# liruiluo/VLA-Adapter

Hardware: AMD Instinct MI355X
Metric: fine-tune samples/sec (224px img + 32-tok prompt), adapter-only, fwd+bwd+AdamW (higher is better)
Workload: dtype bf16

## Files before the change

### vla_adapter_amd/csrc/common.h

```cpp
#pragma once
#include <hip/hip_runtime.h>
#include <stdint.h>
#include <stdio.h>

typedef unsigned short bf16_t;
typedef __attribute__((ext_vector_type(8))) short bf16x8;
typedef __attribute__((ext_vector_type(4))) short bf16x4;
typedef __attribute__((ext_vector_type(4))) float f32x4;
typedef __attribute__((ext_vector_type(16))) float f32x16;
typedef __attribute__((ext_vector_type(4))) unsigned u32x4;
typedef __attribute__((ext_vector_type(8))) int v8i_f8;

#define VLA_OK 0
#define VLA_ERR_ARG (-1)
#define VLA_ERR_LAUNCH (-2)
#define VLA_ERR_UNSUPPORTED (-3)

extern "C" void vla_set_error(const char* msg);

#define VLA_REQUIRE(cond, msg)            \
  do {                                    \
    if (!(cond)) {                        \
      vla_set_error(msg);                 \
      return VLA_ERR_ARG;                 \
// ... 39 lines not shown
}
__device__ __forceinline__ void unpack8(const uint4& u, float (&f)[8]) {
  const unsigned w[4] = {u.x, u.y, u.z, u.w};
#pragma unroll
  for (int k = 0; k < 4; ++k) {
    f[2 * k] = bf_lo(w[k]);
    f[2 * k + 1] = bf_hi(w[k]);
  }
}
template <class V>
__device__ __forceinline__ uint2 pack4(const V& f) { return uint2{pack2(f[0], f[1]), pack2(f[2], f[3])}; }
__device__ __forceinline__ uint4 pack8(const float (&f)[8]) {
  return uint4{pack2(f[0], f[1]), pack2(f[2], f[3]), pack2(f[4], f[5]), pack2(f[6], f[7])};
}

__device__ __forceinline__ unsigned long long splitmix64_key(unsigned long long seed, unsigned long long idx) {
  unsigned long long z = seed + idx * 0x9E3779B97F4A7C15ull;
  z = (z ^ (z >> 30)) * 0xBF58476D1CE4E5B9ull;
  z = (z ^ (z >> 27)) * 0x94D049BB133111EBull;
  return z ^ (z >> 31);
}

__device__ __forceinline__ long long action_token_id(float v, const double* __restrict__ bins, int nbins, float lo, float hi,
                                                     long long tokenizer_len) {
  const double x = (double)fminf(fmaxf(v, lo), hi);
  int a = 0, b = nbins;
  while (a < b) {
    const int mid = (a + b) >> 1;
    if (bins[mid] <= x) a = mid + 1;
    else b = mid;
  }
  return tokenizer_len - a;
}

__device__ __forceinline__ float wave_sum(float v) {
#pragma unroll
  for (int o = 32; o > 0; o >>= 1) v += __shfl_xor(v, o, 64);
  return v;
}
__device__ __forceinline__ float wave_max(float v) {
#pragma unroll
  for (int o = 32; o > 0; o >>= 1) v = fmaxf(v, __shfl_xor(v, o, 64));
  return v;
}

__device__ __forceinline__ float fast_erf(float x) {
  const float ax = fabsf(x);
  const float t = __builtin_amdgcn_rcpf(1.0f + 0.3275911f * ax);
  const float poly = t * (0.254829592f + t * (-0.284496736f + t * (1.421413741f + t * (-1.453152027f + t * 1.061405429f))));
  const float r = 1.0f - poly * __expf(-ax * ax);
  return copysignf(r, x);
}
__device__ __forceinline__ float gelu_erf(float x) {
  const float ax = fabsf(x);
  const float t = __builtin_amdgcn_rcpf(__builtin_fmaf(ax, 0.3275911f * 0.70710678118654752440f, 1.0f));
  const float poly = t * (0.127414796f + t * (-0.142248368f + t * (0.7107068705f + t * (-0.7265760135f + t * 0.5307027145f))));
  const float e = __builtin_amdgcn_exp2f(x * x * -0.72134752044448170368f);
  return __builtin_fmaf(-ax * poly, e, fmaxf(x, 0.f));
}
__device__ __forceinline__ float gelu_erf_grad(float x) {
  const float c = 0.3989422804014327f;
  return 0.5f * (1.0f + fast_erf(x * 0.70710678118654752440f)) + x * c * __expf(-0.5f * x * x);
}
__device__ __forceinline__ float gelu_tanh(float x) {
  const float u2 = x * __builtin_fmaf(x * x, 0.044715f * 1.5957691216057308f, 1.5957691216057308f);
  return x * __builtin_amdgcn_rcpf(1.0f + __builtin_amdgcn_exp2f(u2 * -1.4426950408889634f));
}

__device__ __forceinline__ void lds_zero16(void* p, int bytes, int idx, int n) {
  for (int i = idx * 16; i < bytes; i += n * 16) *reinterpret_cast<uint4*>(reinterpret_cast<char*>(p) + i) = uint4{0, 0, 0, 0};
}

__device__ __forceinline__ void glds16(const void* gptr, void* lds_wave_base) {
  __builtin_amdgcn_global_load_lds((const __attribute__((address_space(1))) void*)gptr,
                                   (__attribute__((address_space(3))) void*)lds_wave_base, 16, 0, 0);
}

__device__ __forceinline__ void glds16s(const char* base, unsigned voff, unsigned dst) {
  unsigned keep;
  asm volatile("s_mov_b32 %0, m0\n\ts_mov_b32 m0, %3\n\ts_nop 0\n\tglobal_load_lds_dwordx4 %1, %2\n\ts_mov_b32 m0, %0"
               : "=&s"(keep) : "v"(voff), "s"(base), "s"(dst) : "memory");
}

__device__ __forceinline__ v8i_f8 cat8(bf16x8 lo, bf16x8 hi) {
  typedef float f32x8 __attribute__((ext_vector_type(8)));
  const f32x4 l = __builtin_bit_cast(f32x4, lo), h = __builtin_bit_cast(f32x4, hi);
  return __builtin_bit_cast(v8i_f8, f32x8{l[0], l[1], l[2], l[3], h[0], h[1], h[2], h[3]});
}

#define VLA_BARRIER()                      \
  do {                                     \
    __builtin_amdgcn_sched_barrier(0);     \
    __builtin_amdgcn_s_barrier();          \
    asm volatile("" ::: "memory");         \
    __builtin_amdgcn_sched_barrier(0);     \
  } while (0)

__device__ __forceinline__ int xcd_order(int bid, int nwg) {
  const int xcd = bid & 7, q8 = nwg >> 3, r8 = nwg & 7;
  return (xcd < r8 ? xcd * (q8 + 1) : r8 * (q8 + 1) + (xcd - r8) * q8) + (bid >> 3);
}

constexpr int CR_THREADS = 1024;

template <int LPR>
struct CR {
  static constexpr int COLS = 8 * LPR, GROUPS = CR_THREADS / LPR;
  static __device__ __forceinline__ int col() { return blockIdx.x * COLS + (threadIdx.x % LPR) * 8; }
  static __device__ __forceinline__ int row0() { return threadIdx.x / LPR; }
  static int blocks(int cols) { return (cols + COLS - 1) / COLS; }

  static __device__ __forceinline__ void add(float (&a)[8], float* __restrict__ out, int cols, float (*sm)[64]) {
    const int lane = threadIdx.x & 63, w = threadIdx.x >> 6;
#pragma unroll
    for (int k = 0; k < 8; ++k)
#pragma unroll
      for (int o = LPR; o < 64; o <<= 1) a[k] += __shfl_xor(a[k], o, 64);
    if (lane < LPR)
#pragma unroll
      for (int k = 0; k < 8; ++k) sm[w][lane * 8 + k] = a[k];
    __syncthreads();
    const int c = blockIdx.x * COLS + threadIdx.x;
    if (threadIdx.x < COLS && c < cols) {
      float s = 0.f;
#pragma unroll
      for (int i = 0; i < CR_THREADS / 64; ++i) s += sm[i][threadIdx.x];
      atomicAdd(out + c, s);
    }
    __syncthreads();
  }
};

#define CR_LAUNCH(KERNEL, rows, cols, batch, stream, ...) \
  hipLaunchKernelGGL(KERNEL<8>, dim3(CR<8>::blocks(cols), 1, (batch)), dim3(CR_THREADS), 0, (hipStream_t)(stream), __VA_ARGS__)
```

### vla_adapter_amd/csrc/elementwise.hip

```cpp
#include "gemm_epilogue.h"
#include "argmax_order.h"
#include <type_traits>

namespace {

inline unsigned nblk(long long n, int per) { return (unsigned)((n + per - 1) / per); }

__global__ void im2col_kernel(const void* __restrict__ px, bf16_t* __restrict__ out, int B, int Ctot, int c0, int H,
                              int W, int P, int ldo, int f32in) {
  const int gw = W / P, gh = H / P, KK = 3 * P * P;
  const long long total = (long long)B * gh * gw * ldo;
  for (long long i = (long long)blockIdx.x * blockDim.x + threadIdx.x; i < total; i += (long long)gridDim.x * blockDim.x) {
    const int col = i % ldo;
    const long long prow = i / ldo;
    float v = 0.f;
    if (col < KK) {
      const int c = col / (P * P), rem = col - c * P * P, py = rem / P, pxx = rem - py * P;
      const int pw = prow % gw, ph = (prow / gw) % gh, b = prow / ((long long)gw * gh);
      const long long src = (((long long)b * Ctot + c0 + c) * H + ph * P + py) * W + pw * P + pxx;
      v = f32in ? ((const float*)px)[src] : bf2f(((const bf16_t*)px)[src]);
    }
    out[i] = f2bf(v);
  }
}

__global__ void action_mask_kernel(const long long* __restrict__ labels, int* __restrict__ qidx, int* __restrict__ pos,
                                   int* __restrict__ count, int B, int L, int shift) {
  const int b = blockIdx.x, lane = threadIdx.x;
  const long long* row = labels + (long long)b * L + shift;
  const int n = L - shift;
  int base = 0;
  for (int j0 = 0; j0 < n; j0 += 64) {
    const int j = j0 + lane;
    const bool sel = j < n && row[j] != -100 && row[j] > 151386;
    const unsigned long long bal = __ballot(sel);
    const int k = base + __popcll(bal & ((1ull << lane) - 1ull));
    if (j < n) qidx[(long long)b * n + j] = sel ? k : -1;
    if (sel && k < 64) pos[b * 64 + k] = j;
    base += __popcll(bal);
  }
  if (lane == 0) count[b] = base;
  for (int k = base + lane; k < 64; k += 64) pos[b * 64 + k] = -1;
}

__global__ void embed_splice_kernel(const long long* __restrict__ ids, const unsigned char* __restrict__ am,
                                    const int* __restrict__ qidx, const bf16_t* __restrict__ table,
                                    const bf16_t* __restrict__ aq, bf16_t* __restrict__ out,
                                    unsigned char* __restrict__ mm, int B, int L, int Np, int D, int vocab) {
  const int S = L + Np;
  const int lane = threadIdx.x & 63;
  const long long r = (long long)blockIdx.x * 4 + (threadIdx.x >> 6);
  if (r >= (long long)B * S) return;
  const int b = r / S, s = r - (long long)b * S;
  if (s >= 1 && s <= Np) {
    if (lane == 0 && mm) mm[r] = 1;
    return;
  }
  const int j = s == 0 ? 0 : s - Np;
  const int qi = qidx[(long long)b * L + j];
  long long id = ids[(long long)b * L + j];
  if (id < 0 || id >= vocab) id = 0;
  const bf16_t* src = qi >= 0 ? aq + (long long)min(qi, 63) * D : table + id * D;
  bf16_t* dst = out + r * D;
  for (int e = lane * 8; e < D; e += 512) *reinterpret_cast<uint4*>(dst + e) = *reinterpret_cast<const uint4*>(src + e);
  if (lane == 0 && mm) mm[r] = am ? (am[(long long)b * L + j] != 0) : 1;
}

__global__ void action_query_grad_kernel(const bf16_t* __restrict__ dx, const int* __restrict__ pos, float* __restrict__ dq,
                                         int B, int S, int Np, int D, int row0) {
  const int k = blockIdx.x;
  for (int d = threadIdx.x; d < D; d += blockDim.x) {
    float a = 0.f;
    for (int b = 0; b < B; ++b) {
      const int j = pos[b * 64 + k];
      if (j < 0) continue;
      const int s = (j == 0 ? 0 : Np + j) - row0;
      if (s < 0) continue;
      a += bf2f(dx[((long long)b * S + s) * D + d]);
    }
    dq[k * D + d] = a;
  }
}

__global__ void gather_rows_kernel(const bf16_t* __restrict__ in, const int* __restrict__ idx, bf16_t* __restrict__ out,
// ... 58 lines not shown
#pragma unroll
    for (int k = 0; k < 8; ++k) {
      const float sg = 1.f / (1.f + __expf(-g[k]));
      du[k] = d[k] * (g[k] * sg);
      dg[k] = d[k] * u[k] * silu_grad(g[k], sg);
    }
    *reinterpret_cast<uint4*>(dgu + go) = pack8(dg);
    *reinterpret_cast<uint4*>(dgu + go + 16) = pack8(du);
  }
}

__global__ __launch_bounds__(256) void transpose_kernel(const bf16_t* __restrict__ in, bf16_t* __restrict__ out, int rows,
                                                        int cols, int ldi, int ldo, long long s_in, long long s_out) {
  __shared__ bf16_t t[64][66];
  const bf16_t* ib = in + (long long)blockIdx.z * s_in;
  bf16_t* ob = out + (long long)blockIdx.z * s_out;
  const int r0 = blockIdx.y * 64, c0 = blockIdx.x * 64;
  const int tx = threadIdx.x & 63, ty = threadIdx.x >> 6;
  for (int r = ty; r < 64; r += 4)
    t[r][tx] = (r0 + r < rows && c0 + tx < cols) ? ib[(long long)(r0 + r) * ldi + c0 + tx] : (bf16_t)0;
  __syncthreads();
  for (int c = ty; c < 64; c += 4)
    if (c0 + c < cols && r0 + tx < rows) ob[(long long)(c0 + c) * ldo + r0 + tx] = t[tx][c];
}

__global__ __launch_bounds__(256) void transpose_vec_kernel(const bf16_t* __restrict__ in, bf16_t* __restrict__ out, int rows,
                                                            int cols, int ldi, int ldo, long long s_in, long long s_out) {
  __shared__ unsigned t32[64 * 33];
  const bf16_t* ib = in + (long long)blockIdx.z * s_in;
  bf16_t* ob = out + (long long)blockIdx.z * s_out;
  const int r0 = blockIdx.y * 64, c0 = blockIdx.x * 64;
  for (int i = threadIdx.x; i < 512; i += 256) {
    const int r = i >> 3, ch = i & 7;
    uint4 v = {0u, 0u, 0u, 0u};
    if (r0 + r < rows && c0 + ch * 8 < cols) v = *reinterpret_cast<const uint4*>(ib + (long long)(r0 + r) * ldi + c0 + ch * 8);
    unsigned* d = t32 + r * 33 + ch * 4;
    d[0] = v.x; d[1] = v.y; d[2] = v.z; d[3] = v.w;
  }
  __syncthreads();
  const bf16_t* t = reinterpret_cast<const bf16_t*>(t32);
  for (int i = threadIdx.x; i < 512; i += 256) {
    const int g = i & 7, c = i >> 3;
    if (c0 + c < cols && r0 + g * 8 < rows) {
      unsigned o[4];
#pragma unroll
      for (int k = 0; k < 4; ++k)
        o[k] = (unsigned)t[(g * 8 + 2 * k) * 66 + c] | ((unsigned)t[(g * 8 + 2 * k + 1) * 66 + c] << 16);
      *reinterpret_cast<uint4*>(ob + (long long)(c0 + c) * ldo + r0 + g * 8) = uint4{o[0], o[1], o[2], o[3]};
    }
  }
}

__global__ void colsum_kernel(const bf16_t* __restrict__ x, float* __restrict__ out, int rows, int cols, int ldx, long long s_x,
                              long long s_out) {
  const int c = blockIdx.x * 256 + threadIdx.x;
  if (c >= cols) return;
  x += (long long)blockIdx.z * s_x;
  out += (long long)blockIdx.z * s_out;
  float a = 0.f;
  for (int r = 0; r < rows; ++r) a += bf2f(x[(long long)r * ldx + c]);
  atomicAdd(out + c, a);
}

template <int LPR>
__global__ __launch_bounds__(CR_THREADS) void colsum_vec_kernel(const bf16_t* __restrict__ x, float* __restrict__ out, int rows, int cols,
                                                                int ldx, long long s_x, long long s_out) {
  __shared__ float sm[CR_THREADS / 64][64];
  const int c = CR<LPR>::col();
  x += (long long)blockIdx.z * s_x;
  out += (long long)blockIdx.z * s_out;
  float a[8] = {0, 0, 0, 0, 0, 0, 0, 0};
  if (c < cols)
    for (int r = CR<LPR>::row0(); r < rows; r += CR<LPR>::GROUPS) {
      float f[8];
      unpack8(*reinterpret_cast<const uint4*>(x + (long long)r * ldx + c), f);
#pragma unroll
      for (int k = 0; k < 8; ++k) a[k] += f[k];
    }
  CR<LPR>::add(a, out, cols, sm);
}

__global__ void cast_f32_bf16_kernel(const float* __restrict__ x, bf16_t* __restrict__ y, long long n) {
  for (long long i = (long long)blockIdx.x * blockDim.x + threadIdx.x; i < n; i += (long long)gridDim.x * blockDim.x) y[i] = f2bf(x[i]);
}
__global__ void cast_bf16_f32_kernel(const bf16_t* __restrict__ x, float* __restrict__ y, long long n) {
  for (long long i = (long long)blockIdx.x * blockDim.x + threadIdx.x; i < n; i += (long long)gridDim.x * blockDim.x) y[i] = bf2f(x[i]);
}

__global__ void rope_half_kernel(bf16_t* __restrict__ x, const float* __restrict__ ct, const float* __restrict__ st, long long rows,
                                 int S, int nheads, int dh, int ldx, float sign) {
  const int half = dh / 2;
  const long long total = rows * nheads * half;
  for (long long i = (long long)blockIdx.x * blockDim.x + threadIdx.x; i < total; i += (long long)gridDim.x * blockDim.x) {
    const int d = i % half;
    const long long t = i / half;
    const int hh = t % nheads;
    const long long r = t / nheads;
    const int pos = r % S;
    bf16_t* p = x + r * ldx + hh * dh + d;
    const float a = bf2f(p[0]), b = bf2f(p[half]);
    const float c = ct[pos * half + d], s = sign * st[pos * half + d];
    p[0] = f2bf(rope_rot_a(a, b, c, s));
    p[half] = f2bf(rope_rot_b(a, b, c, s));
  }
}

__global__ void rope_inter_kernel(bf16_t* __restrict__ x, const float* __restrict__ ct, const float* __restrict__ st,
                                  long long rows, int T, int nheads, int dh, int ldx, int mode) {
  const int half = dh / 2;
  const long long total = rows * nheads * half;
  for (long long i = (long long)blockIdx.x * blockDim.x + threadIdx.x; i < total; i += (long long)gridDim.x * blockDim.x) {
    const int d = i % half;
    const long long t = i / half;
    const int hh = t % nheads;
    const long long r = t / nheads;
    const int pos = r % T;
    bf16_t* p = x + r * ldx + hh * dh + 2 * d;
    const float a = bf2f(p[0]), b = bf2f(p[1]);
    const float ca = ct[pos * dh + 2 * d], cb = ct[pos * dh + 2 * d + 1];
    const float sa = st[pos * dh + 2 * d], sb = st[pos * dh + 2 * d + 1];
    if (mode == 0) {
      p[0] = f2bf(rope_rot_a(a, b, ca, sa));
      p[1] = f2bf(rope_rot_b(a, b, cb, sb));
    } else {
      p[0] = f2bf(a * ca + b * sb);
      p[1] = f2bf(b * cb - a * sa);
    }
  }
}

__global__ void rope_inter_vec_kernel(bf16_t* __restrict__ x, const float* __restrict__ ct, const float* __restrict__ st,
                                      int rows, int T, int nheads, int dh, int ldx, int mode) {
  const int cpr = nheads * dh / 8;
  const long long total = (long long)rows * cpr;
  for (long long i = (long long)blockIdx.x * blockDim.x + threadIdx.x; i < total; i += (long long)gridDim.x * blockDim.x) {
    const int r = (int)(i / cpr), col = (int)(i - (long long)r * cpr) * 8;
    const int d0 = col % dh, pos = r % T;
    uint4* px = reinterpret_cast<uint4*>(x + (long long)r * ldx + col);
    float f[8], o[8];
    unpack8(*px, f);
    const float4 c0 = *reinterpret_cast<const float4*>(ct + (long long)pos * dh + d0), c1 = *reinterpret_cast<const float4*>(ct + (long long)pos * dh + d0 + 4);
    const float4 s0 = *reinterpret_cast<const float4*>(st + (long long)pos * dh + d0), s1 = *reinterpret_cast<const float4*>(st + (long long)pos * dh + d0 + 4);
    const float cc[8] = {c0.x, c0.y, c0.z, c0.w, c1.x, c1.y, c1.z, c1.w}, ss[8] = {s0.x, s0.y, s0.z, s0.w, s1.x, s1.y, s1.z, s1.w};
#pragma unroll
    for (int k = 0; k < 8; k += 2) {
      const float a = f[k], b = f[k + 1];
      if (mode == 0) {
        o[k] = rope_rot_a(a, b, cc[k], ss[k]);
        o[k + 1] = rope_rot_b(a, b, cc[k + 1], ss[k + 1]);
      } else {
        o[k] = a * cc[k] + b * ss[k + 1];
        o[k + 1] = b * cc[k + 1] - a * ss[k];
      }
    }
    *px = pack8(o);
  }
}

__global__ __launch_bounds__(256) void l1_loss_kernel(const bf16_t* __restrict__ pred, const bf16_t* __restrict__ tgt,
                                                      float* __restrict__ loss3, bf16_t* __restrict__ dpred, int B, int C,
                                                      int Da, float gscale) {
  __shared__ float red[3][4];
  const int n = B * C * Da;
  float a = 0.f, cur = 0.f, nxt = 0.f;
  for (int i = threadIdx.x; i < n; i += 256) {
    const float d = bf2f(pred[i]) - bf2f(tgt[i]);
// ... 209 lines not shown
  hipLaunchKernelGGL(action_query_grad_kernel, dim3(64), dim3(256), 0, (hipStream_t)stream, (const bf16_t*)dx, pos, dq, B, S, Np, D, row0);
  VLA_CHECK_LAUNCH("action_query_grad");
  return VLA_OK;
}

extern "C" int vla_gather_rows(void* stream, const void* in, const int* idx, void* out, int n, int D, int ldi, int ldo) {
  VLA_REQUIRE(in && idx && out && n > 0 && D % 8 == 0 && ldi % 8 == 0 && ldo % 8 == 0, "gather_rows: bad args");
  VLA_REQUIRE(((((uintptr_t)in) | ((uintptr_t)out)) & 15) == 0, "gather_rows: 16-B aligned in / out");
  hipLaunchKernelGGL(gather_rows_kernel, dim3(nblk(n, 4)), dim3(256), 0, (hipStream_t)stream, (const bf16_t*)in, idx, (bf16_t*)out, n, D, ldi, ldo);
  VLA_CHECK_LAUNCH("gather_rows");
  return VLA_OK;
}

extern "C" int vla_scatter_add_rows(void* stream, const void* in, const int* idx, void* out, int n, int D, int ldi, int ldo) {
  VLA_REQUIRE(in && idx && out && n > 0 && D % 8 == 0 && ldi % 8 == 0 && ldo % 8 == 0, "scatter_add_rows: bad args");
  VLA_REQUIRE(((((uintptr_t)in) | ((uintptr_t)out)) & 15) == 0, "scatter_add_rows: 16-B aligned in / out");
  hipLaunchKernelGGL(scatter_add_rows_kernel, dim3(nblk(n, 4)), dim3(256), 0, (hipStream_t)stream, (const bf16_t*)in, idx, (bf16_t*)out, n, D, ldi, ldo);
  VLA_CHECK_LAUNCH("scatter_add_rows");
  return VLA_OK;
}

#define EW_ENTRY(NAME, OP, NEEDB)                                                                                  \
  extern "C" int NAME(void* stream, const void* a, const void* b, void* y, long long n) {                           \
    VLA_REQUIRE(a && y && (!(NEEDB) || b) && n > 0 && n % 8 == 0, #NAME ": null / n%8");                              \
    VLA_REQUIRE(((((uintptr_t)a) | ((uintptr_t)b) | ((uintptr_t)y)) & 15) == 0, #NAME ": 16-B aligned tensors");     \
    hipLaunchKernelGGL(ew_kernel<OP>, GRID1D(n / 8, 256), dim3(256), 0, (hipStream_t)stream, (const bf16_t*)a,     \
                       (const bf16_t*)b, (bf16_t*)y, n / 8);                                                       \
    VLA_CHECK_LAUNCH(#NAME);                                                                                       \
    return VLA_OK;                                                                                                 \
  }
EW_ENTRY(vla_add_bf16, EW_ADD, 1)
EW_ENTRY(vla_gelu_bwd, EW_GELU_B, 1)
EW_ENTRY(vla_relu_bwd, EW_RELU_B, 1)
extern "C" int vla_gelu_fwd(void* stream, const void* x, void* y, long long n) {
  VLA_REQUIRE(x && y && n > 0 && n % 8 == 0, "gelu_fwd: null / n%8");
  VLA_REQUIRE(((((uintptr_t)x) | ((uintptr_t)y)) & 15) == 0, "gelu_fwd: 16-B aligned tensors");
  hipLaunchKernelGGL(ew_kernel<EW_GELU_F>, GRID1D(n / 8, 256), dim3(256), 0, (hipStream_t)stream, (const bf16_t*)x,
                     (const bf16_t*)nullptr, (bf16_t*)y, n / 8);
  VLA_CHECK_LAUNCH("gelu_fwd");
  return VLA_OK;
}

extern "C" int vla_swiglu_bwd(void* stream, const void* dh, const void* gu, void* dgu, int M, int I) {
  VLA_REQUIRE(dh && gu && dgu && M > 0 && I > 0 && I % 16 == 0, "swiglu_bwd: I%16");
  VLA_REQUIRE(((((uintptr_t)dh) | ((uintptr_t)gu) | ((uintptr_t)dgu)) & 15) == 0, "swiglu_bwd: 16-B aligned tensors");
  const long long nch = (long long)M * (I / 8);
  hipLaunchKernelGGL(swiglu_bwd_kernel, GRID1D(nch, 256), dim3(256), 0, (hipStream_t)stream, (const bf16_t*)dh, (const bf16_t*)gu, (bf16_t*)dgu, nch, I);
  VLA_CHECK_LAUNCH("swiglu_bwd");
  return VLA_OK;
}

extern "C" int vla_transpose_bf16(void* stream, const void* in, void* out, int rows, int cols, int ldi, int ldo, int batch,
                                  long long s_in, long long s_out) {
  VLA_REQUIRE(in && out && rows > 0 && cols > 0 && ldi >= cols && ldo >= rows && batch > 0, "transpose: bad args");
  dim3 grid((cols + 63) / 64, (rows + 63) / 64, batch);
  const bool vec = rows % 8 == 0 && cols % 8 == 0 && ldi % 8 == 0 && ldo % 8 == 0 && s_in % 8 == 0 && s_out % 8 == 0 &&
                   ((((uintptr_t)in) | ((uintptr_t)out)) & 15) == 0;
  if (vec)
    hipLaunchKernelGGL(transpose_vec_kernel, grid, dim3(256), 0, (hipStream_t)stream, (const bf16_t*)in, (bf16_t*)out, rows, cols, ldi, ldo, s_in, s_out);
  else
    hipLaunchKernelGGL(transpose_kernel, grid, dim3(256), 0, (hipStream_t)stream, (const bf16_t*)in, (bf16_t*)out, rows, cols, ldi, ldo, s_in, s_out);
  VLA_CHECK_LAUNCH("transpose");
  return VLA_OK;
}

extern "C" int vla_colsum_bf16(void* stream, const void* x, float* out, int rows, int cols, int ldx, int batch, long long s_x,
                               long long s_out) {
  VLA_REQUIRE(x && out && rows > 0 && cols > 0 && ldx >= cols && batch > 0, "colsum: bad args");
  if (cols % 8 == 0 && ldx % 8 == 0 && s_x % 8 == 0 && ((uintptr_t)x & 15) == 0) {
    CR_LAUNCH(colsum_vec_kernel, rows, cols, batch, stream, (const bf16_t*)x, out, rows, cols, ldx, s_x, s_out);
    VLA_CHECK_LAUNCH("colsum");
    return VLA_OK;
  }
  hipLaunchKernelGGL(colsum_kernel, dim3((cols + 255) / 256, 1, batch), dim3(256), 0, (hipStream_t)stream, (const bf16_t*)x, out, rows,
                     cols, ldx, s_x, s_out);
  VLA_CHECK_LAUNCH("colsum");
  return VLA_OK;
}

extern "C" int vla_cast_f32_bf16(void* stream, const float* x, void* y, long long n) {
  VLA_REQUIRE(x && y && n > 0, "cast: bad args");
  hipLaunchKernelGGL(cast_f32_bf16_kernel, GRID1D(n, 256), dim3(256), 0, (hipStream_t)stream, x, (bf16_t*)y, n);
  VLA_CHECK_LAUNCH("cast_f32_bf16");
  return VLA_OK;
}
extern "C" int vla_cast_bf16_f32(void* stream, const void* x, float* y, long long n) {
  VLA_REQUIRE(x && y && n > 0, "cast: bad args");
  hipLaunchKernelGGL(cast_bf16_f32_kernel, GRID1D(n, 256), dim3(256), 0, (hipStream_t)stream, (const bf16_t*)x, y, n);
  VLA_CHECK_LAUNCH("cast_bf16_f32");
  return VLA_OK;
}

extern "C" int vla_rope_half(void* stream, void* x, const float* cos_t, const float* sin_t, int rows, int S, int nheads, int dh,
                             int ldx, int sign) {
  VLA_REQUIRE(x && cos_t && sin_t && rows > 0 && S > 0 && nheads > 0 && dh % 2 == 0 && ldx >= nheads * dh, "rope_half: bad args");
  const long long total = (long long)rows * nheads * (dh / 2);
  hipLaunchKernelGGL(rope_half_kernel, GRID1D(total, 256), dim3(256), 0, (hipStream_t)stream, (bf16_t*)x, cos_t, sin_t, (long long)rows, S, nheads, dh, ldx, sign >= 0 ? 1.f : -1.f);
  VLA_CHECK_LAUNCH("rope_half");
  return VLA_OK;
}

extern "C" int vla_rope_interleaved(void* stream, void* x, const float* cos_t, const float* sin_t, int rows, int T, int nheads,
                                    int dh, int ldx, int mode) {
  VLA_REQUIRE(x && cos_t && sin_t && rows > 0 && T > 0 && nheads > 0 && dh % 2 == 0 && ldx >= nheads * dh, "rope_interleaved: bad args");
  const long long total = (long long)rows * nheads * (dh / 2);
  if (dh % 8 == 0 && ldx % 8 == 0 && (((uintptr_t)x | (uintptr_t)cos_t | (uintptr_t)sin_t) & 15) == 0) {
    const long long tv = (long long)rows * (nheads * dh / 8);
    hipLaunchKernelGGL(rope_inter_vec_kernel, GRID1D(tv, 256), dim3(256), 0, (hipStream_t)stream, (bf16_t*)x, cos_t, sin_t, (int)rows, T, nheads, dh, ldx, mode);
  } else
  hipLaunchKernelGGL(rope_inter_kernel, GRID1D(total, 256), dim3(256), 0, (hipStream_t)stream, (bf16_t*)x, cos_t, sin_t, (long long)rows, T, nheads, dh, ldx, mode);
  VLA_CHECK_LAUNCH("rope_interleaved");
  return VLA_OK;
}

extern "C" int vla_l1_loss(void* stream, const void* pred, const void* target, float* loss3, void* dpred, int B, int C, int Da,
                           float gscale) {
  VLA_REQUIRE(pred && target && loss3 && B > 0 && C > 0 && Da > 0, "l1_loss: bad args");
  hipLaunchKernelGGL(l1_loss_kernel, dim3(1), dim3(256), 0, (hipStream_t)stream, (const bf16_t*)pred, (const bf16_t*)target, loss3, (bf16_t*)dpred, B, C, Da, gscale);
  VLA_CHECK_LAUNCH("l1_loss");
  return VLA_OK;
}

static int adamw_launch(void* stream, void* p, const void* g, void* m, void* v, long long n, double lr, double beta1, double beta2,
                        double eps, double wd, int step, int g_f32, float gscale, const float* coef) {
  VLA_REQUIRE(p && g && m && v && n > 0 && step >= 1, "adamw: bad args");
  const double bc1 = 1.0 - pow(beta1, step), bc2 = 1.0 - pow(beta2, step);
  const float decay = (float)(1.0 - lr * wd);
  const float omb1 = (float)(1.0 - beta1), omb2 = (float)(1.0 - beta2);
  const float neg_step = (float)(-(lr / bc1));
  const float gs = gscale == 0.f ? 1.f : gscale;
  const bool aligned = ((((uintptr_t)p) | ((uintptr_t)g) | ((uintptr_t)m) | ((uintptr_t)v)) & 15) == 0;
  const long long n8 = aligned ? n / 8 : 0, done = n8 * 8;
  if (n8 > 0)
    hipLaunchKernelGGL(coef ? adamw_vec8_kernel<true> : adamw_vec8_kernel<false>, GRID1D(n8, 256), dim3(256), 0, (hipStream_t)stream,
                       (uint4*)p, g, (uint4*)m, (uint4*)v, n8, decay, omb1, (float)beta2, omb2, (float)sqrt(bc2), (float)eps, neg_step,
                       g_f32, gs, coef);
  if (done < n)
    hipLaunchKernelGGL(coef ? adamw_kernel<true> : adamw_kernel<false>, GRID1D(n - done, 256), dim3(256), 0, (hipStream_t)stream,
                       (bf16_t*)p + done, g_f32 ? (const void*)((const float*)g + done) : (const void*)((const bf16_t*)g + done),
                       (bf16_t*)m + done, (bf16_t*)v + done, n - done, decay, omb1, (float)beta2, omb2, (float)sqrt(bc2), (float)eps,
                       neg_step, g_f32, gs, coef);
  VLA_CHECK_LAUNCH("adamw");
  return VLA_OK;
}

extern "C" int vla_adamw_bf16(void* stream, void* p, const void* g, void* m, void* v, long long n, double lr, double beta1,
                              double beta2, double eps, double wd, int step, int g_f32, float gscale) {
  return adamw_launch(stream, p, g, m, v, n, lr, beta1, beta2, eps, wd, step, g_f32, gscale, nullptr);
}

extern "C" int vla_adamw_clipped_bf16(void* stream, void* p, const void* g, void* m, void* v, long long n, double lr, double beta1,
                                      double beta2, double eps, double wd, int step, int g_f32, float gscale, const float* coef) {
  VLA_REQUIRE(coef, "adamw_clipped: null coefficient");
  return adamw_launch(stream, p, g, m, v, n, lr, beta1, beta2, eps, wd, step, g_f32, gscale, coef);
}

extern "C" long long vla_grad_sumsq_slots(long long n) { return n > 0 ? (n + GRAD_SSQ_CHUNK - 1) / GRAD_SSQ_CHUNK : 0; }

extern "C" int vla_grad_sumsq(void* stream, const void* g, long long n, int g_f32, float gscale, float* slots) {
  VLA_REQUIRE(g && slots && n > 0, "grad_sumsq: bad args");
  VLA_REQUIRE(((uintptr_t)g & (g_f32 ? 3 : 1)) == 0 && ((uintptr_t)slots & 3) == 0, "grad_sumsq: misaligned pointer");
  const long long nb = vla_grad_sumsq_slots(n);
  VLA_REQUIRE(nb <= 0x7fffffffLL, "grad_sumsq: slice too long");
  const float gs = gscale == 0.f ? 1.f : gscale;
  hipLaunchKernelGGL(g_f32 ? grad_sumsq_kernel<true> : grad_sumsq_kernel<false>, dim3((unsigned)nb), dim3(256), 0, (hipStream_t)stream, g, n, gs, slots);
  VLA_CHECK_LAUNCH("grad_sumsq");
// ... 643 lines not shown
```

### vla_adapter_amd/csrc/gemm.hip

```cpp
#include <algorithm>
#include "gemm_epilogue.h"
#include "gemm_params.h"

namespace {

constexpr int BK = 64;
constexpr int EPI_PAD = 16;

__device__ __forceinline__ float apply_act(float v, int act) {
  switch (act) {
    case VLA_ACT_GELU: return rbf(gelu_erf(v));
    case VLA_ACT_RELU: return fmaxf(v, 0.f);
    case VLA_ACT_GELU_TANH: return rbf(gelu_tanh(v));
    default: return v;
  }
}

template <int BM, int BN, int STAGES, int WN = 2>
struct Cfg {
  static constexpr int NW = (BM / 64) * WN;
  static constexpr int NTHREADS = NW * 64;
  static constexpr int WTN = BN / WN;
  static constexpr int NT = WTN / 16;
  static constexpr int A_BYTES = BM * BK * 2, B_BYTES = BN * BK * 2;
  static constexpr int STAGE_BYTES = A_BYTES + B_BYTES;
  static constexpr int PIECES = STAGE_BYTES / 1024;
  static constexpr int PPW = PIECES / NW;
  static constexpr int EPI_STRIDE = WTN * 2 + EPI_PAD;
  static constexpr int LDS_BYTES = STAGES * STAGE_BYTES;
  static constexpr int NHALF = NW * 64 * EPI_STRIDE <= LDS_BYTES ? 1 : 2;
  static constexpr int EPI_ROWS = 64 / NHALF;
  static constexpr int EPI_BYTES = NW * EPI_ROWS * EPI_STRIDE;
  static_assert(EPI_BYTES <= LDS_BYTES, "epilogue staging must fit the operand ring");
  static_assert(PIECES % NW == 0, "pieces must divide evenly over the waves");
};

template <int BM, int BN, int STAGES, int ROPE, int WN = 2, bool F8 = false, bool EXT = false>
__global__ __launch_bounds__((BM / 64) * 64 * WN) __attribute__((amdgpu_waves_per_eu((F8 && EXT) ? 4 : 1)))
void gemm_nt_kernel(GemmP p) {
  using C = Cfg<BM, BN, STAGES, WN>;
  constexpr int EB = F8 ? 1 : 2;
  extern __shared__ __attribute__((aligned(16))) char smem[];
  const int tid = threadIdx.x, lane = tid & 63;
  const int wid = __builtin_amdgcn_readfirstlane(tid >> 6);
  const int wr = wid / WN, wc = wid - wr * WN;

  const int swz = xcd_order(blockIdx.x, p.ntiles);
  constexpr int GM = 6;
  const int tiles_m = p.ntiles / p.tiles_n, per_group = GM * p.tiles_n;
  const int grp = swz / per_group, rem = swz - grp * per_group;
  const int gm = min(GM, tiles_m - grp * GM);
  const int bm = grp * GM + rem % gm, bn = rem / gm;
  const int m0 = bm * BM, n0 = bn * BN;
  const int z = blockIdx.z;
  const char* Ab = reinterpret_cast<const char*>(p.A) + (long long)z * p.sA * EB;
  const char* Bb = reinterpret_cast<const char*>(p.B) + (long long)z * p.sB * EB;

  const int kc = ((lane & 7) ^ ((lane >> 3) & 7)) * 16;
  const char* pp[C::PPW];
#pragma unroll
  for (int i = 0; i < C::PPW; ++i) {
    const int pc = wid * C::PPW + i;
    if (pc < BM / 8) {
      const int ra = min(m0 + pc * 8 + (lane >> 3), p.M - 1);
      pp[i] = Ab + grouped_row(ra, p.gA, p.sgA, p.lda) * EB + kc;
    } else {
      const int rb = min(n0 + (pc - BM / 8) * 8 + (lane >> 3), p.N - 1);
      pp[i] = Bb + (long long)rb * p.ldb * EB + kc;
    }
  }
  const char* pp2[EXT ? C::PPW : 1];
  if constexpr (EXT) {
#pragma unroll
    for (int i = 0; i < C::PPW; ++i) {
      const int pc = wid * C::PPW + i;
      if (pc < BM / 8) pp2[i] = reinterpret_cast<const char*>(p.A2) + (long long)min(m0 + pc * 8 + (lane >> 3), p.M - 1) * p.lda2 * 2 + kc;
      else pp2[i] = reinterpret_cast<const char*>(p.B2) + (long long)min(n0 + (pc - BM / 8) * 8 + (lane >> 3), p.N - 1) * p.ldb2 * 2 + kc;
    }
  }
  const int nt1 = (p.Ktot > 0 ? min(p.K, p.Ktot - z * p.K) : p.K) / (F8 ? 2 * BK : BK);
  auto stage = [&](int buf, int t) {
    char* base = smem + buf * C::STAGE_BYTES + wid * C::PPW * 1024;
    if (EXT && t >= nt1) {
#pragma unroll
      for (int i = 0; i < C::PPW; ++i) glds16(pp2[i] + (t - nt1) * 128, base + i * 1024);
    } else {
#pragma unroll
      for (int i = 0; i < C::PPW; ++i) glds16(pp[i] + t * 128, base + i * 1024);
    }
  };

  f32x4 acc[C::NT][4];
#pragma unroll
  for (int a = 0; a < C::NT; ++a)
#pragma unroll
    for (int b = 0; b < 4; ++b) acc[a][b] = f32x4{0.f, 0.f, 0.f, 0.f};

  const int frow = lane & 15;
  int foff[2], foff2[2];
#pragma unroll
  for (int s = 0; s < 2; ++s) {
    foff[s] = frow * 128 + (((F8 ? 2 * (lane >> 4) + s : 4 * s + (lane >> 4)) ^ (lane & 7)) << 4);
    foff2[s] = frow * 128 + (((4 * s + (lane >> 4)) ^ (lane & 7)) << 4);
  }

  const int wm0 = m0 + wr * 64, wn0 = n0 + wc * C::WTN;
  const int lq = lane >> 4, lr = lane & 15;
  constexpr bool PERM = ROPE == 1 && C::NT == 2;
  const bool wide = PERM && p.rope_dh == 128;
  auto cbase = [&](int ni) { return PERM ? (wide ? ni * 64 + wc * 16 : (wc >> 1) * 64 + ni * 32 + (wc & 1) * 16) : wc * C::WTN + ni * 16; };
  const bf16_t* bias = p.bias ? p.bias + (long long)z * p.sBias : nullptr;
  float bv[C::NT][4];
  {
    const bool bvec = bias && (((size_t)bias & 7) == 0);
#pragma unroll
    for (int ni = 0; ni < C::NT; ++ni) {
      const int n = n0 + cbase(ni) + lq * 4;
      if (bvec && n + 3 < p.N) {
        const uint2 b2 = *reinterpret_cast<const uint2*>(bias + n);
        bv[ni][0] = bf_lo(b2.x); bv[ni][1] = bf_hi(b2.x);
        bv[ni][2] = bf_lo(b2.y); bv[ni][3] = bf_hi(b2.y);
      } else {
#pragma unroll
        for (int j = 0; j < 4; ++j) bv[ni][j] = (bias && n + j < p.N) ? bf2f(bias[n + j]) : 0.f;
      }
    }
  }

  const int nt = nt1 + (EXT ? p.K2 / BK : 0);
#pragma unroll
  for (int s = 0; s < STAGES - 1; ++s)
    if (s < nt) stage(s, s);
  int buf = 0;
  static_assert(C::NT <= 4, "wave tiles are 64 x 32 or 64 x 64");
  static_assert(STAGES >= 2 && STAGES <= 6 && 4 * C::PPW < 64, "the counted waits below cover rings of 2 to 6 stages (vmcnt is a 6-bit counter)");
#define VLA_KTILE(F8T, FO)                                                                                                           \
  do {                                                                                                                               \
           \
    if (STAGES >= 6 && t + 4 < nt) asm volatile("s_waitcnt vmcnt(%0)" ::"n"(4 * C::PPW) : "memory");                                  \
    else if (STAGES >= 5 && t + 3 < nt) asm volatile("s_waitcnt vmcnt(%0)" ::"n"(3 * C::PPW) : "memory");                             \
    else if (STAGES >= 4 && t + 2 < nt) asm volatile("s_waitcnt vmcnt(%0)" ::"n"(2 * C::PPW) : "memory");                             \
    else if (STAGES >= 3 && t + 1 < nt) asm volatile("s_waitcnt vmcnt(%0)" ::"n"(C::PPW) : "memory");                                 \
    else asm volatile("s_waitcnt vmcnt(0)" ::: "memory");                                                                            \
    __builtin_amdgcn_s_barrier();                     \
    asm volatile("" ::: "memory");                                                                                                   \
    if (t + STAGES - 1 < nt) {                                                                                                       \
      int nb = buf + STAGES - 1;                                                                                                     \
      if (nb >= STAGES) nb -= STAGES;                                                                                                \
      stage(nb, t + STAGES - 1);                                                                                                     \
    }                                                                                                                                \
    const char* sa = smem + buf * C::STAGE_BYTES + wr * 64 * 128;                                                                    \
    const char* sb = smem + buf * C::STAGE_BYTES + C::A_BYTES;              \
    bf16x8 fm[2][4], fn[2][C::NT];                                                                                                   \
    _Pragma("unroll") for (int s = 0; s < 2; ++s) {                                                                                  \
      _Pragma("unroll") for (int i = 0; i < 4; ++i) fm[s][i] = *reinterpret_cast<const bf16x8*>(sa + i * 16 * 128 + FO[s]);          \
      _Pragma("unroll") for (int i = 0; i < C::NT; ++i) fn[s][i] = *reinterpret_cast<const bf16x8*>(sb + cbase(i) * 128 + FO[s]);    \
    }                                                                                                                                \
    if constexpr (F8T) {                                                                                                             \
      _Pragma("unroll") for (int ni = 0; ni < C::NT; ++ni)                                                                           \
        _Pragma("unroll") for (int mi = 0; mi < 4; ++mi)                                                                             \
          acc[ni][mi] = __builtin_amdgcn_mfma_scale_f32_16x16x128_f8f6f4(cat8(fn[0][ni], fn[1][ni]), cat8(fm[0][mi], fm[1][mi]),     \
                                                                         acc[ni][mi], 0, 0, 0, 0x7f7f7f7f, 0, 0x7f7f7f7f);            \
    } else {                                                                                                                         \
      _Pragma("unroll") for (int s = 0; s < 2; ++s)                                                                                  \
        _Pragma("unroll") for (int ni = 0; ni < C::NT; ++ni)                                                                         \
          _Pragma("unroll") for (int mi = 0; mi < 4; ++mi)                                                                           \
            acc[ni][mi] = __builtin_amdgcn_mfma_f32_16x16x32_bf16(fn[s][ni], fm[s][mi], acc[ni][mi], 0, 0, 0);                       \
    }                                                                                                                                \
    if (++buf == STAGES) buf = 0;                                                                                                    \
  } while (0)
  if constexpr (F8 && EXT) {
    for (int t = 0; t < nt1; ++t) VLA_KTILE(true, foff);
    {
      float fsa[4];
#pragma unroll
      for (int mi = 0; mi < 4; ++mi) fsa[mi] = p.scaleA[min(wm0 + mi * 16 + lr, p.M - 1)];
#pragma unroll
      for (int ni = 0; ni < C::NT; ++ni)
#pragma unroll
        for (int j = 0; j < 4; ++j) {
          const float sbv = p.scaleB[min(n0 + cbase(ni) + lq * 4 + j, p.N - 1)];
#pragma unroll
          for (int mi = 0; mi < 4; ++mi) acc[ni][mi][j] *= fsa[mi] * sbv;
        }
    }
    for (int t = nt1; t < nt; ++t) VLA_KTILE(false, foff2);
  } else {
    for (int t = 0; t < nt; ++t) VLA_KTILE(F8, foff);
  }
#undef VLA_KTILE
  asm volatile("s_waitcnt lgkmcnt(0)" ::: "memory");
  __builtin_amdgcn_s_barrier();
  asm volatile("" ::: "memory");

  if constexpr (F8 && !EXT) {
    float sa[4];
#pragma unroll
    for (int mi = 0; mi < 4; ++mi) sa[mi] = p.scaleA[min(wm0 + mi * 16 + lr, p.M - 1)];
#pragma unroll
    for (int ni = 0; ni < C::NT; ++ni) {
      const int n = n0 + cbase(ni) + lq * 4;
#pragma unroll
      for (int j = 0; j < 4; ++j) {
        const float sbv = p.scaleB[min(n + j, p.N - 1)];
#pragma unroll
        for (int mi = 0; mi < 4; ++mi) acc[ni][mi][j] *= sa[mi] * sbv;
      }
    }
  }
  if (ROPE == 0 && p.ws != nullptr) {
    float* plane = p.ws + (long long)z * p.M * p.N;
#pragma unroll
    for (int ni = 0; ni < C::NT; ++ni)
#pragma unroll
      for (int mi = 0; mi < 4; ++mi) {
        const int m = wm0 + mi * 16 + lr, n = wn0 + ni * 16 + lq * 4;
        if (m < p.M && n + 3 < p.N)
          *reinterpret_cast<f32x4*>(plane + (long long)m * p.N + n) = acc[ni][mi];
      }
    return;
  }
  char* reg = smem + wid * (C::EPI_ROWS * C::EPI_STRIDE);

  if (ROPE == 3) {
    const bf16_t* GU = p.R + (long long)z * p.sR;
    bf16_t* Cb = p.C + (long long)z * p.sC;
    constexpr int ROWB = 2 * C::WTN * 2 + 16;
    constexpr int CH2 = 2 * C::WTN / 8, RPP2 = 64 / CH2;
    constexpr int NIT = 32 / RPP2;
    char* reg2 = smem + wid * (32 * ROWB);
    if (wn0 >= p.N || wm0 >= p.M) return;
    u32x4 gin[2][NIT];
#pragma unroll
    for (int half = 0; half < 2; ++half)
#pragma unroll
      for (int it = 0; it < NIT; ++it) {
        const int row = it * RPP2 + lane / CH2, ch = lane % CH2;
        const int m = min(wm0 + half * 32 + row, p.M - 1);
        gin[half][it] = *reinterpret_cast<const u32x4*>(GU + grouped_row(m, p.gR, p.sgR, p.ldr) + 2 * wn0 + ch * 8);
// ... 136 lines not shown
            const int row = it * RPP + row0;
            const uint4 v = *reinterpret_cast<const uint4*>(reg + row * C::EPI_STRIDE + ch * 16);
            *reinterpret_cast<uint4*>(Cb + (long long)(wmh + row) * p.ldc + n) = add_packed8(v, rv[it]);
          }
        } else {
#pragma unroll
          for (int it = 0; it < NIT; ++it) {
            const int row = it * RPP + row0;
            *reinterpret_cast<uint4*>(Cb + (long long)(wmh + row) * p.ldc + n) = *reinterpret_cast<const uint4*>(reg + row * C::EPI_STRIDE + ch * 16);
          }
        }
        continue;
      }
    }
#pragma unroll
    for (int it = 0; it < C::EPI_ROWS / RPP; ++it) {
      const int row = it * RPP + lane / CH, ch = lane % CH;
      const int m = wm0 + half * C::EPI_ROWS + row, n = n0 + cbase(ch >> 1) + (ch & 1) * 8;
      uint4 v = *reinterpret_cast<const uint4*>(reg + row * C::EPI_STRIDE + ch * 16);
      if (m >= p.M || n >= p.N) continue;
      if (!row_live(m, p.c_live_mod, p.c_live_from)) continue;
      const long long roff = residual_row(m, p.res_mod, p.gR, p.sgR, p.ldr);
      const long long crow = grouped_row(m, p.gC, p.sgC, p.ldc);
      if (vec_ok && n + 8 <= p.N) {
        if (Rb) v = add_packed8(v, *reinterpret_cast<const uint4*>(Rb + roff + n));
        *reinterpret_cast<uint4*>(Cb + crow + n) = v;
      } else {
        const unsigned wv[4] = {v.x, v.y, v.z, v.w};
#pragma unroll
        for (int k = 0; k < 8; ++k) {
          if (n + k < p.N) {
            float f = (k & 1) ? bf_hi(wv[k >> 1]) : bf_lo(wv[k >> 1]);
            if (Rb) f += bf2f(Rb[roff + n + k]);
            Cb[crow + n + k] = f2bf(f);
          }
        }
      }
    }
  }
}

__global__ void splitk_finalize_kernel(const float* __restrict__ ws, const bf16_t* __restrict__ bias, const bf16_t* __restrict__ R,
                                       bf16_t* __restrict__ C, int M, int N, int ldc, int ldr, int act, float alpha, int split, int vec) {
  const long long total = (long long)M * N / 4, plane = (long long)M * N;
  for (long long i = (long long)blockIdx.x * blockDim.x + threadIdx.x; i < total; i += (long long)gridDim.x * blockDim.x) {
    const int m = (int)(i * 4 / N), n = (int)(i * 4 - (long long)m * N);
    f32x4 pv[8];
#pragma unroll
    for (int z = 0; z < 8; ++z) pv[z] = z < split ? *reinterpret_cast<const f32x4*>(ws + z * plane + i * 4) : f32x4{0.f, 0.f, 0.f, 0.f};
    uint2 braw = {0, 0}, rraw = {0, 0};
    if (vec) {
      if (bias) braw = *reinterpret_cast<const uint2*>(bias + n);
      if (R) rraw = *reinterpret_cast<const uint2*>(R + (long long)m * ldr + n);
    } else {
      if (bias) braw = uint2{(unsigned)bias[n] | ((unsigned)bias[n + 1] << 16), (unsigned)bias[n + 2] | ((unsigned)bias[n + 3] << 16)};
      if (R) {
        const bf16_t* rp = R + (long long)m * ldr + n;
        rraw = uint2{(unsigned)rp[0] | ((unsigned)rp[1] << 16), (unsigned)rp[2] | ((unsigned)rp[3] << 16)};
      }
    }
    f32x4 a = pv[0];
#pragma unroll
    for (int z = 1; z < 8; ++z) a += pv[z];
    for (int z = 8; z < split; ++z) a += *reinterpret_cast<const f32x4*>(ws + z * plane + i * 4);
    const float bb[4] = {bf_lo(braw.x), bf_hi(braw.x), bf_lo(braw.y), bf_hi(braw.y)};
    const float rr[4] = {bf_lo(rraw.x), bf_hi(rraw.x), bf_lo(rraw.y), bf_hi(rraw.y)};
    float o[4];
#pragma unroll
    for (int j = 0; j < 4; ++j) {
      float v = epi_linear(a[j], alpha, bias ? bb[j] : 0.f);
      if (act != VLA_ACT_NONE) v = apply_act(rbf(v), act);
      if (R) v = rbf(v) + rr[j];
      o[j] = v;
    }
    if (vec) {
      *reinterpret_cast<uint2*>(C + (long long)m * ldc + n) = pack4(o);
    } else {
#pragma unroll
      for (int j = 0; j < 4; ++j) C[(long long)m * ldc + n + j] = f2bf(o[j]);
    }
  }
}

template <int BM, int BN, int STAGES, int ROPE, int WN = 2, bool F8 = false, bool EXT = false>
int launch(const GemmP& p0, int nb, hipStream_t st) {
  using C = Cfg<BM, BN, STAGES, WN>;
  if (int rc = vla_lds_limit<gemm_nt_kernel<BM, BN, STAGES, ROPE, WN, F8, EXT>>(C::LDS_BYTES, "gemm_nt_kernel")) return rc;
  GemmP p = p0;
  p.tiles_n = (p.N + BN - 1) / BN;
  p.ntiles = ((p.M + BM - 1) / BM) * p.tiles_n;
  hipLaunchKernelGGL((gemm_nt_kernel<BM, BN, STAGES, ROPE, WN, F8, EXT>), dim3(p.ntiles, 1, nb), dim3(C::NTHREADS), C::LDS_BYTES, st, p);
  return VLA_OK;
}

template <int ROPE, bool F8 = false, bool EXT = false>
int launch_nt(int kernel, const GemmP& p, int nb, hipStream_t st) {
  if constexpr (!F8 && !EXT && ROPE != 3) {
    if (kernel == VLA_KERNEL_NT_64x128_S6) return launch<64, 128, 6, ROPE, 4>(p, nb, st);
    if (kernel == VLA_KERNEL_NT_128x128_S4) return launch<128, 128, 4, ROPE, 4>(p, nb, st);
    if constexpr (ROPE != 1)
      if (kernel == VLA_KERNEL_NT_128x64) return launch<128, 64, 2, ROPE>(p, nb, st);
  }
  return launch<128, 128, 2, ROPE, 4, F8, EXT>(p, nb, st);
}

struct NtOverrides {
  int tile;
  bool no_skinny, no_small_rows, no_splitk, grid_set;
  long long grid;
};
NtOverrides nt_overrides() {
  const char* tile = getenv("VLA_GEMM_TILE");
  const char* nsk = getenv("VLA_NO_SPLITK");
  const char* grid = getenv("VLA_GEMM256_GRID");
  return {tile ? atoi(tile) : 0, getenv("VLA_NO_SKINNY") != nullptr, getenv("VLA_NO_SMALL_ROWS") != nullptr, nsk && *nsk,
          grid != nullptr, grid ? atoll(grid) : 0};
}

thread_local int g_latency_hint = 0;

bool use_256(int M, int N, int K, int batch, int act, int ncu) {
  const long long tiles = (long long)((M + 255) / 256) * ((N + 255) / 256) * batch;
  if (act == VLA_ACT_SWIGLU_BWD) return false;
  if ((act == VLA_ACT_GELU || act == VLA_ACT_GELU_TANH) && tiles > ncu && (tiles % ncu) != 0 && (tiles % ncu) * 4 < ncu) return false;
  const long long t128 = (long long)((M + 127) / 128) * ((N + 127) / 128) * batch;
  const double est256 = (double)((tiles + ncu - 1) / ncu) * 4.0, est128 = (double)((t128 + 2 * ncu - 1) / (2 * ncu)) * (2.0 / 0.87);
  return M >= 1024 && N >= 768 && K >= 256 && est256 < est128;
}

int skinny_tile(const vla_gemm_desc* d, bool latency, int ncu, bool no_small_rows) {
  const bool tall = (d->N == 64 || d->N == 128 || d->N == 192) && d->M >= 1024;
  const bool shortm = latency && d->M <= 512 && d->N % 16 == 0 && d->K >= 512 && !no_small_rows;
  if (!(tall || shortm) || d->K % 128 != 0 || d->K >= 2048 || d->ldc % 8 != 0 || ((uintptr_t)d->C & 15) != 0) return -1;
  if (!(d->act == VLA_ACT_NONE || d->act == VLA_ACT_GELU || d->act == VLA_ACT_RELU || d->act == VLA_ACT_GELU_TANH)) return -1;
  if (d->bias && ((uintptr_t)d->bias & 15) != 0) return -1;
  if (d->R && (d->ldr % 8 != 0 || ((uintptr_t)d->R & 15) != 0)) return -1;
  if ((d->rope_mode == 1 && (d->rope_dh != 64 || d->rope_cols % 64 != 0 || tall)) ||
      (d->rope_mode == 2 && (d->rope_dh % 8 != 0 || d->rope_cols % 8 != 0 || (((uintptr_t)d->rope_cos | (uintptr_t)d->rope_sin) & 15) != 0)))
    return -1;
  int best = -1;
  long long best_cost = 0;
  for (int t = 0; t < SKINNY_TILES; ++t) {
    const int tm = 16 * SKINNY_TILE[t][0], tn = 16 * SKINNY_TILE[t][1];
    if (tall && d->N % tn != 0) continue;
    if (d->rope_mode == 1 && tn != 64) continue;
    const long long wgs = (long long)((d->M + tm - 1) / tm) * ((d->N + tn - 1) / tn), cost = (long long)(tm + tn) * ((wgs + ncu - 1) / ncu);
    if (best < 0 || cost < best_cost || (cost == best_cost && t > best)) best = t, best_cost = cost;
  }
  if (!tall && best_cost > 96) return -1;
  return best;
}

bool ext_on_256(const vla_gemm_desc* d, int force, int ncu) {
  if (d->fp8 || d->batch != 1 || d->split_k > 1 || d->act == VLA_ACT_SWIGLU_BWD || d->rope_mode == 2 || d->a_group != 0 ||
      (d->rope_mode == 1 && d->rope_dh != 64) || !vla_gemm256_extent_ok(d))
    return false;
  const unsigned long long ra = (unsigned long long)((d->M + 255) / 256) * 256, rb = (unsigned long long)((d->N + 255) / 256) * 256;
  if ((ra * d->lda2 + d->K2) * 2 >= (1ull << 32) || (rb * d->ldb2 + d->K2) * 2 >= (1ull << 32)) return false;
  if (force != 0) return force == 6;
  const long long t256 = (long long)((d->M + 255) / 256) * ((d->N + 255) / 256);
  if (d->rope_mode == 1 && t256 < 192) return false;
  return use_256(d->M, d->N, d->K + d->K2, 1, d->act, ncu);
}

struct NtPlan { int kernel, split; };

NtPlan plan_nt(const vla_gemm_desc* d, bool latency, int ncu, const NtOverrides& ov) {
  const int force = ov.tile, kt = d->K / BK;
  const int asked = d->split_k > 1 ? d->split_k : 1, per = (kt + asked - 1) / asked, split = (kt + per - 1) / per;
  if (force == 0 && !ov.no_skinny && d->batch == 1 && split == 1 && d->a_group == 0 && d->c_group == 0 && d->r_group == 0 &&
      d->res_mod == 0 && d->c_live_mod == 0 && !d->fp8 && d->K2 == 0 && d->C) {
    const int t = skinny_tile(d, latency, ncu, ov.no_small_rows);
    if (t >= 0) return {VLA_KERNEL_NT_SKINNY + t, 1};
  }
  const bool fits256 = vla_gemm256_extent_ok(d) != 0;
  if (d->K2 > 0) return {!d->fp8 && ext_on_256(d, force, ncu) ? VLA_KERNEL_NT_256 : VLA_KERNEL_NT_128x128, 1};
  if (d->fp8) {
    const bool big = force == 6 || (force == 0 && d->M >= 4096 && d->N >= 4096 && d->K >= 4096);
    return {big && d->c_group == 0 && d->r_group == 0 && fits256 && !(d->rope_mode == 1 && d->rope_dh != 64) ? VLA_KERNEL_NT_256
                                                                                                              : VLA_KERNEL_NT_128x128, 1};
  }
  const int nb = asked > 1 ? asked : d->batch;
  bool square = false;
  if (asked == 1) {
    const long long t256 = (long long)((d->M + 255) / 256) * ((d->N + 255) / 256) * nb;
    if (force == 6 || (force == 0 && (d->rope_mode == 0 || t256 >= 192) && use_256(d->M, d->N, d->K, nb, d->act, ncu))) {
      if (fits256 && !(d->rope_mode == 2 && (d->R || d->act != VLA_ACT_NONE)) && !(d->rope_mode == 1 && d->rope_dh != 64))
        return {VLA_KERNEL_NT_256, 1};
      square = true;
    }
  }
  if (d->act == VLA_ACT_SWIGLU_BWD) return {VLA_KERNEL_NT_128x128, split};
  const long long tiles = (long long)((d->M + 127) / 128) * ((d->N + 127) / 128) * nb;
  const bool narrow = !square && d->rope_mode != 1 && force != 2 && (force == 3 || (tiles <= 128 && d->K / asked >= 4096 && d->N % 64 == 0));
  if (narrow) return {VLA_KERNEL_NT_128x64, split};
  if (latency && per >= 4) {
    const int runs = split > 1 ? split : d->batch;
    const long long wgs = (long long)((d->M + 127) / 128) * ((d->N + 127) / 128) * runs, wgs64 = (long long)((d->M + 63) / 64) * ((d->N + 127) / 128) * runs;
    if (wgs64 <= ncu) return {VLA_KERNEL_NT_64x128_S6, split};
    if (wgs <= ncu) return {VLA_KERNEL_NT_128x128_S4, split};
  }
  return {VLA_KERNEL_NT_128x128, split};
}

int auto_split_k(const vla_gemm_desc* d, bool latency, int ncu, const NtOverrides& ov) {
  const bool plain = !d->fp8 && d->K2 == 0 && d->batch == 1 && !d->bias_post_round && d->C && d->a_group == 0 && d->c_group == 0 &&
                     d->r_group == 0 && d->rope_mode == 0 && d->c_live_mod == 0 && d->res_mod == 0 && d->N % 4 == 0 &&
                     (d->act == VLA_ACT_NONE || d->act == VLA_ACT_GELU || d->act == VLA_ACT_RELU || d->act == VLA_ACT_GELU_TANH);
  if (!plain || d->K < 2048 || ov.no_splitk) return 1;
  const long long tiles = (long long)((d->M + 127) / 128) * ((d->N + 127) / 128), t64 = (long long)((d->M + 63) / 64) * ((d->N + 127) / 128);
  if (latency && t64 * 2 <= ncu) return (int)std::max(2LL, std::min({ncu / t64, (long long)(d->K / BK) / 4, 16LL}));
  if (tiles > ncu) return 1;
  for (int sk = 8; sk >= 2; sk /= 2)
    if (tiles * sk <= 2 * ncu && d->K % (BK * sk) == 0 && d->K / sk >= 512) return sk;
  return 1;
}

int splitk_finalize(const vla_gemm_desc* d, int split, hipStream_t st) {
  const long long total = (long long)d->M * d->N / 4;
  const unsigned nblk = (unsigned)((total + 255) / 256 < 2048 ? (total + 255) / 256 : 2048);
  hipLaunchKernelGGL(splitk_finalize_kernel, dim3(nblk), dim3(256), 0, st, (const float*)d->ws, (const bf16_t*)d->bias,
                     (const bf16_t*)d->R, (bf16_t*)d->C, d->M, d->N, d->ldc, d->ldr, d->act, d->alpha == 0.f ? 1.f : d->alpha, split,
                     (d->ldc % 4 == 0 && ((uintptr_t)d->C & 7) == 0 && (!d->R || (d->ldr % 4 == 0 && ((uintptr_t)d->R & 7) == 0)) &&
                      (!d->bias || ((uintptr_t)d->bias & 7) == 0)) ? 1 : 0);
  VLA_CHECK_LAUNCH("gemm_splitk_finalize");
  return VLA_OK;
}

}

extern "C" int vla_gemm256_extent_ok(const vla_gemm_desc* d) {
  if (!d || d->M <= 0 || d->N <= 0 || d->K <= 0) return 0;
  const unsigned long long EB = d->fp8 ? 1 : 2, lim = 1ull << 32;
  const unsigned long long ra = (unsigned long long)((d->M + 255) / 256) * 256 - 1, rb = (unsigned long long)((d->N + 255) / 256) * 256 - 1;
  const unsigned long long offA = d->a_group > 0 ? (ra / d->a_group) * (unsigned long long)d->a_group_stride + (ra % d->a_group) * (unsigned long long)d->lda
                                                 : ra * (unsigned long long)d->lda;
  const unsigned long long offB = rb * (unsigned long long)d->ldb;
  return (offA + d->K) * EB < lim && (offB + d->K) * EB < lim;
}

extern "C" int vla_gemm_latency_hint(int on) {
  const int prev = g_latency_hint;
  if (on >= 0) g_latency_hint = on ? 1 : 0;
  return prev;
}

extern "C" int vla_gemm_nt_plan(const vla_gemm_desc* d, int latency, int num_cus, int* split) {
  if (!d || d->M <= 0 || d->N <= 0 || d->K < BK || d->batch <= 0) return VLA_ERR_ARG;
  const bool lat = latency < 0 ? g_latency_hint > 0 : latency > 0;
  const int ncu = num_cus > 0 ? num_cus : vla_num_cus();
  const NtOverrides ov = nt_overrides();
  const NtPlan pl = plan_nt(d, lat, ncu, ov);
  if (split) *split = d->split_k > 1 ? pl.split : auto_split_k(d, lat, ncu, ov);
  return pl.kernel;
}

extern "C" int vla_gemm_bf16_nt(void* stream, const vla_gemm_desc* d) {
  VLA_REQUIRE(d && d->A && d->B, "gemm: null operand");
  VLA_REQUIRE(d->M > 0 && d->N > 0 && d->K > 0 && d->batch > 0, "gemm: empty problem");
  VLA_REQUIRE(d->K % BK == 0, "gemm: K must be a multiple of 64 (pad the operands)");
  VLA_REQUIRE(d->lda % 8 == 0 && d->ldb % 8 == 0, "gemm: lda/ldb must be multiples of 8 elements (16-B rows)");
  if (d->fp8)
    VLA_REQUIRE(d->fp8 == 1 && d->a_scale && d->b_scale && d->K % 128 == 0 && d->lda % 16 == 0 && d->ldb % 16 == 0 && d->batch == 1 &&
                    d->split_k <= 1 && d->rope_mode != 2 && d->a_group == 0 && (d->act != VLA_ACT_SWIGLU_BWD || d->K2 > 0),
                "gemm: fp8 needs scales, K % 128 == 0, 16-B rows, batch 1, no split-K / interleaved RoPE / row groups on A (SwiGLU backward: with a K extension only)");
  VLA_REQUIRE(((uintptr_t)d->A & 15) == 0 && ((uintptr_t)d->B & 15) == 0, "gemm: A/B must be 16-B aligned");
  VLA_REQUIRE(d->sA % 8 == 0 && d->sB % 8 == 0, "gemm: batch strides of A/B must keep 16-B alignment");
  if (d->act == VLA_ACT_SWIGLU_BWD) {
    VLA_REQUIRE(d->C && d->R && !d->bias && d->rope_mode == 0 && d->N % 64 == 0 && d->ldc % 8 == 0 && d->ldr % 4 == 0 &&
                    ((uintptr_t)d->R & 7) == 0 && d->c_group == 0 && d->res_mod == 0,
                "gemm: swiglu_bwd needs C = dGU [M, 2N] (ldc%8), R = GU [M, 2N] (interleaved), N%64 == 0");
  } else if (d->act == VLA_ACT_SWIGLU) {
    VLA_REQUIRE(d->C2 && d->N % 32 == 0 && d->ldc2 % 4 == 0 && ((uintptr_t)d->C2 & 7) == 0 && d->sC2 % 4 == 0,
                "gemm: swiglu needs C2, N%32==0, ldc2%4==0");
    VLA_REQUIRE(!d->R, "gemm: swiglu epilogue takes no residual");
  } else {
    VLA_REQUIRE(d->C, "gemm: null C");
  }
  if (d->C) VLA_REQUIRE(((uintptr_t)d->C & 15) == 0 || (d->ldc % 8) != 0, "gemm: C must be 16-B aligned");
  if (d->C && d->ldc % 8 == 0) VLA_REQUIRE(d->sC % 8 == 0, "gemm: sC must keep 16-B alignment");
  if (d->R && d->ldc % 8 == 0 && d->ldr % 8 == 0 && d->act != VLA_ACT_SWIGLU_BWD)
    VLA_REQUIRE(((uintptr_t)d->R & 15) == 0 && d->sR % 8 == 0, "gemm: R must be 16-B aligned");
  VLA_REQUIRE(d->a_group >= 0 && d->c_group >= 0 && d->a_group_stride % 8 == 0 &&
                  (d->c_group == 0 || d->ldc % 8 != 0 || d->c_group_stride % 8 == 0),
              "gemm: row-group strides must keep 16-B alignment");
  const bool split_k = d->split_k > 1;
  VLA_REQUIRE(d->bias_post_round == 0 || (d->bias_post_round == 1 && d->bias && d->rope_mode != 1 && !split_k && d->act == VLA_ACT_NONE),
              "gemm: bias_post_round needs a bias and a plain epilogue (no rotate_half rope / split-K / activation)");
  if (split_k) {
    VLA_REQUIRE(d->ws && d->batch == 1 && d->rope_mode == 0 && d->c_group == 0 && d->r_group == 0 &&
                    d->res_mod == 0 && d->c_live_mod == 0 && d->C &&
                    (d->act == VLA_ACT_NONE || d->act == VLA_ACT_GELU || d->act == VLA_ACT_RELU || d->act == VLA_ACT_GELU_TANH),
                "gemm: split_k needs an fp32 workspace [split_k, M, N], batch 1 and a plain epilogue");
    VLA_REQUIRE(d->N % 4 == 0 && ((uintptr_t)d->ws & 15) == 0, "gemm: split_k needs N % 4 == 0 and a 16-B aligned workspace");
  }
  VLA_REQUIRE(d->c_live_mod >= 0 && d->c_live_from >= 0 && (d->c_live_mod == 0 || d->c_live_from < d->c_live_mod),
              "gemm: c_live_from must lie inside c_live_mod");
  VLA_REQUIRE(d->r_group >= 0 && d->r_group_stride % 8 == 0 && (d->r_group == 0 || d->res_mod == 0),
              "gemm: r_group stride must keep 16-B alignment; r_group and res_mod are exclusive");
  if (d->K2 != 0)
    VLA_REQUIRE(d->K2 > 0 && d->K2 % BK == 0 && d->A2 && d->B2 && d->lda2 % 8 == 0 && d->ldb2 % 8 == 0 && (((uintptr_t)d->A2 | (uintptr_t)d->B2) & 15) == 0 &&
                    d->batch == 1 && !split_k && d->rope_mode != 2,
                "gemm: the K extension needs A2 / B2 (bf16, 16-B aligned rows, K2 % 64 == 0), batch 1, no split-K / interleaved RoPE");
  if (d->rope_mode != 0) {
    VLA_REQUIRE(d->rope_mode == 1 || d->rope_mode == 2, "gemm: rope_mode 0/1/2");
    VLA_REQUIRE(d->rope_cos && d->rope_sin && d->rope_T > 0 && d->rope_dh > 0 && d->rope_dh % 4 == 0 && d->rope_cols % 64 == 0 &&
                    (((uintptr_t)d->rope_cos | (uintptr_t)d->rope_sin) & 15) == 0 && d->act != VLA_ACT_SWIGLU,
                "gemm: bad rope arguments");
    if (d->rope_mode == 1) VLA_REQUIRE(d->rope_dh == 64 || (d->rope_dh == 128 && d->N % 128 == 0 && d->rope_cols % 128 == 0),
                                       "gemm: fused rotate_half RoPE needs head dim 64, or 128 with N and rope_cols multiples of 128");
  }

  const NtOverrides ov = nt_overrides();
  const int ncu = vla_num_cus();
  const NtPlan pl = plan_nt(d, g_latency_hint > 0, ncu, ov);

  GemmP p;
  p.A = (const bf16_t*)d->A; p.B = (const bf16_t*)d->B; p.C = (bf16_t*)d->C;
  p.bias = (const bf16_t*)d->bias; p.R = (const bf16_t*)d->R; p.C2 = (bf16_t*)d->C2;
  p.M = d->M; p.N = d->N; p.K = d->K; p.lda = d->lda; p.ldb = d->ldb; p.ldc = d->ldc; p.ldr = d->ldr;
  p.ldc2 = d->ldc2; p.res_mod = d->res_mod; p.act = d->act;
  p.sA = d->sA; p.sB = d->sB; p.sC = d->sC; p.sR = d->sR; p.sC2 = d->sC2; p.sBias = d->sBias;
  p.tiles_n = p.ntiles = 0; p.batch = 1; p.stagger = 0;
  p.alpha = d->alpha == 0.f ? 1.f : d->alpha;
  p.gA = d->a_group; p.sgA = d->a_group_stride; p.gC = d->c_group; p.sgC = d->c_group_stride;
  p.gR = d->r_group; p.sgR = d->r_group_stride;
  p.c_live_mod = d->c_live_mod; p.c_live_from = d->c_live_from;
  p.bias_post = d->bias_post_round;
  p.ws = nullptr; p.Ktot = 0;
  if (split_k) {
    const int kt = d->K / BK;
    p.ws = d->ws;
    p.K = (kt + pl.split - 1) / pl.split * BK;
    p.Ktot = d->K;
    p.sA = p.sB = p.K;
    p.bias = nullptr; p.R = nullptr;
  }
  p.rope_mode = d->rope_mode; p.rope_T = d->rope_T; p.rope_dh = d->rope_dh; p.rope_cols = d->rope_cols;
  p.rope_cos = d->rope_cos; p.rope_sin = d->rope_sin;
  p.scaleA = d->fp8 ? d->a_scale : nullptr; p.scaleB = d->fp8 ? d->b_scale : nullptr;
  p.A2 = (const bf16_t*)d->A2; p.B2 = (const bf16_t*)d->B2; p.K2 = d->K2; p.lda2 = d->lda2; p.ldb2 = d->ldb2;

  hipStream_t st = (hipStream_t)stream;
  const int nb = pl.split > 1 ? pl.split : d->batch;
  const int rope = d->act == VLA_ACT_SWIGLU_BWD ? 3 : d->rope_mode;
  int rc;
  if (pl.kernel < VLA_KERNEL_NT_SKINNY + SKINNY_TILES) rc = vla_gemm_skinny_launch(p, pl.kernel - VLA_KERNEL_NT_SKINNY, st);
  else if (pl.kernel == VLA_KERNEL_NT_256)
    rc = vla_gemm256_launch(p, d->act == VLA_ACT_SWIGLU ? 1 : d->act == VLA_ACT_SWIGLU_BWD ? 2 : 0, d->batch, ov.grid_set ? ov.grid : ncu, st);
  else if (d->K2 > 0 && d->fp8)
    rc = rope == 3 ? launch_nt<3, true, true>(pl.kernel, p, nb, st) : rope == 1 ? launch_nt<1, true, true>(pl.kernel, p, nb, st)
                                                                                : launch_nt<0, true, true>(pl.kernel, p, nb, st);
  else if (d->K2 > 0)
    rc = rope == 3 ? launch_nt<3, false, true>(pl.kernel, p, nb, st) : rope == 1 ? launch_nt<1, false, true>(pl.kernel, p, nb, st)
                                                                                 : launch_nt<0, false, true>(pl.kernel, p, nb, st);
  else if (d->fp8) rc = rope == 1 ? launch_nt<1, true>(pl.kernel, p, nb, st) : launch_nt<0, true>(pl.kernel, p, nb, st);
  else if (rope == 3) rc = launch_nt<3>(pl.kernel, p, nb, st);
  else if (rope == 2) rc = launch_nt<2>(pl.kernel, p, nb, st);
  else if (rope == 1) rc = launch_nt<1>(pl.kernel, p, nb, st);
  else rc = launch_nt<0>(pl.kernel, p, nb, st);
  if (rc) return rc;
  VLA_CHECK_LAUNCH("gemm_bf16_nt");
  if (pl.split > 1) return splitk_finalize(d, pl.split, st);
  return VLA_OK;
}
```

### vla_adapter_amd/csrc/gemm_tn.hip

```cpp
#include <algorithm>
#include "gemm_epilogue.h"
#include "gemm_params.h"

namespace {

constexpr int TBK = 64;
constexpr int TILE_BYTES = TBK * 256;
constexpr int STAGE_BYTES = 2 * TILE_BYTES;
constexpr int LDS_BYTES = 2 * STAGE_BYTES;

struct TnP {
  const bf16_t* A; const bf16_t* B; bf16_t* C; const bf16_t* R; float* ws;
  int M, N1, N2, lda, ldb, ldc, ldr;
  long long sA, sB, sC, sR;
  float alpha;
  int gA, gB; long long sgA, sgB;
  int cgA, cgsA;
  int tiles_n2, ntiles, split, mslice;
};

__device__ __forceinline__ bf16x4 tr_read(const char* p) {
  return __builtin_amdgcn_ds_read_tr16_b64_v4i16((__attribute__((address_space(3))) bf16x4*)p);
}

__device__ __forceinline__ void tn_tile(const TnP& p, const int swz, const int bz, char* smem) {
  const int tid = threadIdx.x, lane = tid & 63;
  const int wid = __builtin_amdgcn_readfirstlane(tid >> 6);
  const int wr = wid >> 2, wc = wid & 3;
  const int b1 = swz / p.tiles_n2, b2 = swz - b1 * p.tiles_n2;
  const int n1_0 = b1 * 128, n2_0 = b2 * 128;
  const int zb = bz / p.split, zs = bz - zb * p.split;
  const int m_begin = zs * p.mslice, m_end = min(p.M, m_begin + p.mslice);
  const int nt = (m_end - m_begin + TBK - 1) / TBK;
  const char* Ab = reinterpret_cast<const char*>(p.A + (long long)zb * p.sA);
  const char* Bb = reinterpret_cast<const char*>(p.B + (long long)zb * p.sB);

  const bool isA = wid < 4;
  const int ld = isA ? p.lda : p.ldb, ncols = isA ? p.N1 : p.N2, c0 = isA ? n1_0 : n2_0;
  const int grp = isA ? p.gA : p.gB;
  const long long sgrp = isA ? p.sgA : p.sgB;
  const char* base = isA ? Ab : Bb;
  int rloc[4];
  long long coff[4];
#pragma unroll
  for (int i = 0; i < 4; ++i) {
    const int qp = (wid & 3) * 4 + i;
    const int r = 4 * qp + (lane >> 4);
    const int f = ((r & 3) << 2) | ((r >> 2) & 3);
    int col = c0 + (((lane & 15) ^ f) << 3);
    col = min(col, ncols - 8);
    if (isA && p.cgA > 0) col = (col / p.cgA) * p.cgsA + col % p.cgA;
    rloc[i] = r;
    coff[i] = (long long)col * 2;
  }
  auto stage = [&](int buf, int t) {
    const int mt = m_begin + t * TBK;
    const long long tb = grouped_row(mt, grp, sgrp, ld);
    const int lim = m_end - 1 - mt;
    char* dst = smem + buf * STAGE_BYTES + (isA ? 0 : TILE_BYTES) + (wid & 3) * 4096;
#pragma unroll
    for (int i = 0; i < 4; ++i) glds16(base + (tb + (long long)min(rloc[i], lim) * ld) * 2 + coff[i], dst + i * 1024);
  };

  const int kq = lane >> 4, qq = (lane >> 2) & 3, pp = lane & 3;
  int fa[4][2], fb[2][2];
#pragma unroll
  for (int e = 0; e < 2; ++e) {
    const int row = 8 * kq + qq + 4 * e, f = (qq << 2) | ((2 * kq + e) & 3);
#pragma unroll
    for (int i = 0; i < 4; ++i) fa[i][e] = 256 * row + ((((wr * 64 + i * 16) >> 3) + (pp >> 1)) ^ f) * 16 + 8 * (pp & 1);
#pragma unroll
    for (int i = 0; i < 2; ++i) fb[i][e] = TILE_BYTES + 256 * row + ((((wc * 32 + i * 16) >> 3) + (pp >> 1)) ^ f) * 16 + 8 * (pp & 1);
  }

  f32x4 acc[2][4];
#pragma unroll
  for (int a = 0; a < 2; ++a)
#pragma unroll
    for (int b = 0; b < 4; ++b) acc[a][b] = f32x4{0.f, 0.f, 0.f, 0.f};

  if (nt > 0) stage(0, 0);
  int buf = 0;
  for (int t = 0; t < nt; ++t) {
    asm volatile("s_waitcnt vmcnt(0)" ::: "memory");
    __builtin_amdgcn_s_barrier();
    asm volatile("" ::: "memory");
    if (t + 1 < nt) stage(buf ^ 1, t + 1);
    const char* sb = smem + buf * STAGE_BYTES;
    const int valid = m_end - (m_begin + t * TBK);
    bf16x8 fm[2][4], fn[2][2];
#pragma unroll
    for (int ks = 0; ks < 2; ++ks) {
#pragma unroll
      for (int i = 0; i < 4; ++i) {
        const bf16x4 lo = tr_read(sb + ks * 8192 + fa[i][0]), hi = tr_read(sb + ks * 8192 + fa[i][1]);
        fm[ks][i] = bf16x8{lo[0], lo[1], lo[2], lo[3], hi[0], hi[1], hi[2], hi[3]};
      }
#pragma unroll
      for (int i = 0; i < 2; ++i) {
        const bf16x4 lo = tr_read(sb + ks * 8192 + fb[i][0]), hi = tr_read(sb + ks * 8192 + fb[i][1]);
        fn[ks][i] = bf16x8{lo[0], lo[1], lo[2], lo[3], hi[0], hi[1], hi[2], hi[3]};
      }
    }
    if (valid < TBK) {
#pragma unroll
      for (int ks = 0; ks < 2; ++ks)
// ... 430 lines not shown
```

### vla_adapter_amd/engine.py

```python
from __future__ import annotations

import contextlib
import math
import os
from dataclasses import dataclass, field
from typing import Dict, List, Optional, Tuple

import torch

from . import ops, schedule
from .ops import ACT_GELU, ACT_GELU_TANH, ACT_NONE, ACT_RELU, ACT_SWIGLU, BF16
from .schedule import Segment, capture_graph, chunks, turnaround_chunks

NUM_TOKENS = 64
IGNORE_INDEX = -100


def rup(n: int, m: int) -> int:
    return (n + m - 1) // m * m


def copy_flat(dst: torch.Tensor, src: torch.Tensor):
    n = src.numel()
    ops.copy2d(src, dst, 1, n, n, n)
# ... 489 lines not shown
        Mr, tv, win = B * R, lin.trains_vectors, self._win
        L, k, d = self.layers[i], f"llm.{i}.", self._d
        _, n2, h = self._keeps(i)
        if self.per_layer:
            d1_out, d_out = self.G_d1[i], (self.G_res[i - 1] if i > 0 else self.d_last)[:Mr]
            d_gu, d_qkv = self.G_gu[i][:Mr], self.G_qkv[i][:Mr]
        else:
            d1_out, d_out, d_gu, d_qkv = self.d_b[:Mr], d, self.d_gu[:Mr], self.d_qkv[:Mr]
        if i < self._n_run - 1:
            ops.add_(d, dHS[i + 1].view(Mr, D))
        tap = lin.taps.get(("llm", i)) if lin.taps is not None else None
        if tap is not None:
            tap["d_out"] = d.clone()
        d_gu = lin._lin_bwd(k + "down", d, h, L["wdT"], out=d_gu, swiglu_gu=self.GU[i][r0:], **({"gu_group": (R, S * 2 * I)} if win else {}))
        d_n = lin._lin_bwd(k + "gu", d_gu, n2, L["wguT"], out=self.G_n2[i] if tv else self.d_n[:Mr])
        if tv:
            lin._defer(lambda dy=d_n, x=self.X1[i], r=self.R2[i], acc=lin.A(k + "n2"): ops.rmsnorm_dw(dy, x, r, acc))
        d1 = ops.rmsnorm_bwd(d_n, self.X1[i], L["n2"], self.R2[i], dres=d, out=d1_out, x_rows=win)
        dao = lin._lin_bwd(k + "o", d1, self.AO[i], L["woT"], out=self.d_n[:Mr])
        q, kk, v = self._attn_views(self.QKV[i].view(B, S, -1))
        dq, dk, dv = self._attn_views(d_qkv.view(B, R, -1))
        ops.attn_bwd(dao.view(B, R, -1), q[:, r0:], kk, v, self.AO[i].view(B, S, -1)[:, r0:], self.LSE[i], H, KV, dh, True,
                     self.kmask, dq=dq, dk=dk, dv=dv, rope=(self.cos, self.sin) if dh in (64, 128) else None, row0=r0)
        if dh not in (64, 128):
            cs, sn = self.cos[r0:], self.sin[r0:]
            ops.rope_half_(d_qkv[:, :H * dh], cs, sn, R, H, dh, sign=-1)
            ops.rope_half_(d_qkv[:, H * dh:(H + KV) * dh], cs, sn, R, KV, dh, sign=-1)
        d_n = lin._lin_bwd(k + "qkv", d_qkv, self._keeps(i)[0], L["wqkvT"], out=self.G_n1[i] if tv else self.d_n[:Mr])
        if tv:
            lin._defer(lambda dy=d_qkv, acc=lin.A(k + "bqkv"): ops.colsum_(dy, acc))
            lin._defer(lambda dy=d_n, x=self.HS[i].view(M, D), r=self.R1[i], acc=lin.A(k + "n1"): ops.rmsnorm_dw(dy, x, r, acc))
        self._d = ops.rmsnorm_bwd(d_n, self.HS[i].view(M, D), L["n1"], self.R1[i], dres=d1, out=d_out, x_rows=win)
        if tap is not None:
            tap["d_in"] = self._d.clone()

    def bwd_result(self) -> torch.Tensor:
        return self._d.view(self.B, self.Rl, self.cfg.d)


class FlatParams:

    def __init__(self, spec: List[Tuple[str, Tuple[int, ...]]], device):
        self.offsets, off = {}, 0
        for name, shape in spec:
            n = math.prod(shape)
            self.offsets[name] = (off, shape)
            off += rup(n, 8)
        self.numel = off
        self.data = torch.zeros(off, device=device, dtype=BF16)
        self.grad = torch.zeros(off, device=device, dtype=BF16)
        self.m = torch.zeros(off, device=device, dtype=BF16)
        self.v = torch.zeros(off, device=device, dtype=BF16)

    def view(self, name, buf=None):
        off, shape = self.offsets[name]
        return (self.data if buf is None else buf)[off:off + math.prod(shape)].view(shape)

    def g(self, name):
        return self.view(name, self.grad)


class Head(_BufferSets):

    H = 8

    def __init__(self, cfg: VLACfg, device):
        self.cfg, self.device, self.pro = cfg, device, cfg.pro
        D, nb, Da, Pd = cfg.llm.d, cfg.num_blocks, cfg.action_dim, cfg.proprio_dim
        assert D % 64 == 0 and (D // self.H) % 8 == 0
        self.D, self.nb, self.Din = D, nb, Da * D
        assert self.Din % 64 == 0
        seg = [("w_adp", (nb, 2 * D, D)), ("b_adp", (nb, 2 * D)),
               ("w_task", (nb, 2 * D, D)), ("b_task", (nb, 2 * D))] if cfg.pro else []
        spec = [("w_x", (nb, 3 * D, D)), ("b_x", (nb, 3 * D))] + seg + [
                ("w_o", (nb, D, D)), ("b_o", (nb, D)), ("w_ffn", (nb, D, D)), ("b_ffn", (nb, D)),
                ("ln_w", (nb, D)), ("ln_b", (nb, D)), ("gate", (nb, 8)),
                ("ln1_w", (self.Din,)), ("ln1_b", (self.Din,)), ("fc1_w", (D, self.Din)), ("fc1_b", (D,)),
                ("ln2_w", (D,)), ("ln2_b", (D,)), ("fc2_w", (Da, D)), ("fc2_b", (Da,)),
                ("p_fc1_w", (D, Pd)), ("p_fc1_b", (D,)), ("p_fc2_w", (D, D)), ("p_fc2_b", (D,)),
                ("action_queries", (NUM_TOKENS, D))]
        self.P = FlatParams(spec, device)
        self.film = {}
        z = lambda *s: torch.zeros(*s, device=device, dtype=BF16)
        self.T = dict(w_x=z(nb, D, 3 * D), w_o=z(nb, D, D), w_ffn=z(nb, D, D), p_fc2_w=z(D, D))
        if cfg.pro:
            self.T.update(w_adp=z(nb, D, 2 * D), w_task=z(nb, D, 2 * D))
        self.fc2T = z(D, 64)
        self.pfc1_pad = z(D, 64)
        self.dirty = True
        self.rope_tab = None
        self.ref_softmax = bool(int(os.environ.get("VLA_HEAD_REF_SOFTMAX", "0")))

    _BLK_PRO = [("q_proj", "w_x", "b_x", 0), ("k_self", "w_x", "b_x", 1), ("v_self", "w_x", "b_x", 2),
                ("k_adapter", "w_adp", "b_adp", 0), ("v_adapter", "w_adp", "b_adp", 1),
                ("k_task", "w_task", "b_task", 0), ("v_task", "w_task", "b_task", 1),
                ("o_proj", "w_o", "b_o", 0), ("ffn.1", "w_ffn", "b_ffn", 0)]
    _BLK_ORIG = [("q_proj", "w_x", "b_x", 0), ("k_proj", "w_x", "b_x", 1), ("v_proj", "w_x", "b_x", 2),
                 ("o_proj", "w_o", "b_o", 0), ("ffn.1", "w_ffn", "b_ffn", 0)]

    @property
    def _BLK(self):
        return self._BLK_PRO if self.pro else self._BLK_ORIG

    def _kv(self, which: str, i: int):
        D = self.D
        if self.pro:
            return self.P.view("w_" + which)[i], self.P.view("b_" + which)[i], self.T["w_" + which][i]
        return self.P.view("w_x")[i, D:], self.P.view("b_x")[i, D:], self.T["w_x"][i][:, D:]

    def named_views(self, buf=None) -> Dict[str, torch.Tensor]:
        P, D, out = self.P, self.D, {}
        v = lambda n: P.view(n, buf)
        for i in range(self.nb):
            pre = f"model.mlp_resnet_blocks.{i}."
            for name, w, b, k in self._BLK:
                out[pre + name + ".weight"] = v(w)[i, k * D:(k + 1) * D]
                out[pre + name + ".bias"] = v(b)[i, k * D:(k + 1) * D]
            out[pre + "ffn.0.weight"], out[pre + "ffn.0.bias"] = v("ln_w")[i], v("ln_b")[i]
            out[pre + "gating_factor"] = v("gate")[i, :1]
        for a, b in (("model.layer_norm1.weight", "ln1_w"), ("model.layer_norm1.bias", "ln1_b"), ("model.fc1.weight", "fc1_w"),
                     ("model.fc1.bias", "fc1_b"), ("model.layer_norm2.weight", "ln2_w"), ("model.layer_norm2.bias", "ln2_b"),
                     ("model.fc2.weight", "fc2_w"), ("model.fc2.bias", "fc2_b")):
            out[a] = v(b)
        return out

    def proprio_views(self, buf=None):
        v = lambda n: self.P.view(n, buf)
        return {"fc1.weight": v("p_fc1_w"), "fc1.bias": v("p_fc1_b"), "fc2.weight": v("p_fc2_w"), "fc2.bias": v("p_fc2_b")}

    def load_state_dicts(self, head_sd: Dict[str, torch.Tensor], proprio_sd: Dict[str, torch.Tensor],
                         action_queries: Optional[torch.Tensor] = None):
        nv = self.named_views()
        for k, t in nv.items():
            t.copy_(head_sd[k].to(self.device, BF16).reshape(t.shape))
        for k, t in head_sd.items():
            if "film_gen" in k:
                self.film[k] = t.to(self.device, BF16)
        for k, t in self.proprio_views().items():
            t.copy_(proprio_sd[k].to(self.device, BF16))
        if action_queries is not None:
            self.P.view("action_queries").copy_(action_queries.to(self.device, BF16))
        self.dirty = True

    def head_state_dict(self):
        sd = {k: v.clone() for k, v in self.named_views().items()}
        sd.update(self.film)
        return sd

    @property
    def dirty(self) -> bool:
        return self._stale_fwd or self._stale_bwd

    @dirty.setter
    def dirty(self, v: bool):
        self._stale_fwd = self._stale_bwd = bool(v)

    def refresh_forward_operands(self):
        if self._stale_fwd:
            pd = self.cfg.proprio_dim
            ops.copy2d(self.P.view("p_fc1_w"), self.pfc1_pad, self.D, pd, pd, self.pfc1_pad.stride(0))
            self._stale_fwd = False

    def refresh_transposes(self):
        if not self._stale_bwd:
            return
        P = self.P
        for k in (("w_x", "w_adp", "w_task", "w_o", "w_ffn") if self.pro else ("w_x", "w_o", "w_ffn")):
            ops.transpose(P.view(k), out=self.T[k])
        ops.transpose(P.view("p_fc2_w"), out=self.T["p_fc2_w"])
        ops.transpose(P.view("fc2_w"), out=self.fc2T)
        self._stale_bwd = False

    def build_buffer_set(self, B: int, Kt: int) -> dict:
        D, nb, T, dev = self.D, self.nb, self.cfg.chunk, self.device
        Ka = NUM_TOKENS + 1
        e = lambda *s, dt=BF16: torch.empty(*s, device=dev, dtype=dt)
        z = lambda *s, dt=BF16: torch.zeros(*s, device=dev, dtype=dt)
        R = B * T
        b = dict(Ka=Ka, Kt=Kt, R=R, h_adp=e(nb, B, Ka, D),
                 KV_adp=e(nb, B * Ka, 2 * D), KV_task=e(nb, B * Kt, 2 * D), dKV_adp=e(nb, B * Ka, 2 * D), dKV_task=e(nb, B * Kt, 2 * D),
                 X=e(nb + 1, R, D),
                 QKVx=e(nb, R, 3 * D), dQKVx=e(nb, R, 3 * D), AOx=e(nb, R, D), O2=e(nb, R, D), LNo=e(nb, R, D), dO2=e(nb, R, D), dFF=e(nb, R, D),
                 probs=e(nb, B, self.H, T, T + Ka + Kt, dt=torch.float32), stats=e(nb, R, 2, dt=torch.float32))
        bkeys = tuple(k for k in ("b_x", "b_adp", "b_task", "b_o", "b_ffn", "fc1_b", "fc2_b", "p_fc1_b", "p_fc2_b") if k in self.P.offsets)
        shapes = [("dgate", (nb,)), ("ln_dw", (nb, D)), ("ln_db", (nb, D)), ("ln1_dw", (self.Din,)), ("ln1_db", (self.Din,)),
                  ("ln2_dw", (D,)), ("ln2_db", (D,)), ("d_pf", (B, D))] + [("b:" + k, tuple(self.P.offsets[k][1])) for k in bkeys]
        acc32 = b["acc32"] = z(sum(rup(math.prod(sh), 4) for _, sh in shapes), dt=torch.float32)
        off, views = 0, {}
        for name, sh in shapes:
            views[name] = acc32[off:off + math.prod(sh)].view(sh)
            off += rup(math.prod(sh), 4)
        b.update({k: views[k] for k in ("dgate", "ln_dw", "ln_db", "ln1_dw", "ln1_db", "ln2_dw", "ln2_db")}, b_f32={k: views["b:" + k] for k in bkeys}, d_pf32=views["d_pf"])
        i32 = lambda: torch.empty(B, Ka, device=dev, dtype=torch.int32)
        b.update(
            row_idx_ka=i32(), row_idx_live_ka=i32(), _idx_scratch=i32(), guard=torch.zeros(1, device=dev, dtype=torch.float32),
            x_in=z(R, self.Din), pr_in=z(B, 64),
            h_task_c=e(nb, B * Kt, D) if Kt % 64 else None,
            dfc2=e(64, D), dpfc1=e(D, 64),
            dh_adp=e(nb, B * Ka, D), dpad=z(R, 64), rope_tab=ops.rope_inter_tables(max(T, Ka, Kt), D // self.H, dev),
            _buf_key=(B, Kt), _prep_key=None)
        return b

    def forward(self, HS: torch.Tensor, pos1: torch.Tensor, proprio: torch.Tensor, Np: int,
                noise: Optional[torch.Tensor] = None) -> torch.Tensor:
        self.fwd_begin(HS, pos1, proprio, Np, noise)
        for i in range(self.nb):
            self.fwd_layer(i)
        return self.fwd_end()

    _FWD_FIELDS = ("HSref", "Np", "S", "B", "pos1", "_prep_key")

    def fwd_begin(self, HS, pos1, proprio, Np, noise=None):
        cfg, P = self.cfg, self.P
        B, S = HS.shape[1], HS.shape[2]
        T = cfg.chunk
        self._alloc(B, Np)
        self.refresh_forward_operands()
        self.HSref, self.Np, self.S, self.B, self.pos1 = HS, Np, S, B, pos1
        assert proprio.dim() == 2 and proprio.stride(1) == 1 and proprio.dtype in (BF16, torch.float32)
        ops.copy2d(proprio, self.pr_in, B, cfg.proprio_dim, proprio.stride(0), 64)
        self.pp_pre = ops.gemm_nt(self.pr_in, self.pfc1_pad, bias=P.view("p_fc1_b"))
        self.pp_act = ops.gelu_fwd(self.pp_pre)
        self.pf = ops.gemm_nt(self.pp_act, P.view("p_fc2_w"), bias=P.view("p_fc2_b"))
        ops.head_index_prep(pos1, pos1, pos1, self.row_idx_ka, self._idx_scratch, None, B, S, Np, 0)
        ops.copy2d(self.pf, self.h_adp[0, 0, NUM_TOKENS], self.nb * B, self.D, self.D, self.Ka * self.D, src_mod=B)
        if noise is not None:
            assert tuple(noise.shape) == (T, self.Din) and noise.is_contiguous()
            ops.copy2d(noise, self.x_in, B * T, self.Din, self.Din, self.Din, src_mod=T)
        else:
            ops.zero_(self.x_in)
        self.x_ln, self.st1 = ops.layernorm_fwd(self.x_in, P.view("ln1_w"), P.view("ln1_b"), 1e-5, want_stats=True)
        ops.gemm_nt(self.x_ln, P.view("fc1_w"), bias=P.view("fc1_b"), act=ACT_RELU, out=self.X[0])

    def fwd_layer(self, i: int):
        cfg, P, D, H = self.cfg, self.P, self.D, self.H
        HS, B, S, Kt, Ka, T = self.HSref, self.B, self.S, self.Kt, self.Ka, cfg.chunk
        dh = D // H
        rc, rs_ = self.rope_tab
        hs2 = HS[i + 1].view(B * S, D)
        ops.gather_rows(hs2, self.row_idx_ka.view(-1), self.h_adp[i].view(B * Ka, D))
        fuse = self.pro and D % 64 == 0 and not os.environ.get("VLA_NO_KV_ROPE_FUSE")
        wa, ba, _ = self._kv("adp", i)
        ops.gemm_nt(self.h_adp[i].view(B * Ka, D), wa, bias=ba, out=self.KV_adp[i], rope=(2, rc, rs_, Ka, dh, D) if fuse else None)
        wt, bt, _ = self._kv("task", i)
        ops.gemm_nt(hs2[:B * Kt], wt, bias=bt, out=self.KV_task[i], a_group=(Kt, S * D), bias_post_round=B > 1,
                    rope=(2, rc, rs_, Kt, dh, D) if fuse else None)
        x = self.X[i]
        if self.pro:
            if not fuse:
                ops.rope_inter_(self.KV_adp[i][:, :D], rc, rs_, Ka, H, dh, 0)
                ops.rope_inter_(self.KV_task[i][:, :D], rc, rs_, Kt, H, dh, 0)
            ops.gemm_nt(x, P.view("w_x")[i], bias=P.view("b_x")[i], out=self.QKVx[i], rope=(2, rc, rs_, T, dh, 2 * D))
        else:
            ops.gemm_nt(x, P.view("w_x")[i], bias=P.view("b_x")[i], out=self.QKVx[i])
        self._attn(i, fwd=True)
        ops.gemm_nt(self.AOx[i], P.view("w_o")[i], bias=P.view("b_o")[i], residual=x, out=self.O2[i])
        ops.layernorm_fwd(self.O2[i], P.view("ln_w")[i], P.view("ln_b")[i], 1e-5, out=self.LNo[i], stats=self.stats[i])
        ops.gemm_nt(self.LNo[i], P.view("w_ffn")[i], bias=P.view("b_ffn")[i], act=ACT_RELU, out=self.X[i + 1])

    def fwd_end(self) -> torch.Tensor:
        P, nb = self.P, self.nb
        self.xf_ln, self.st2 = ops.layernorm_fwd(self.X[nb], P.view("ln2_w"), P.view("ln2_b"), 1e-5, want_stats=True)
        self.pred = ops.gemm_nt(self.xf_ln, P.view("fc2_w"), bias=P.view("fc2_b"))
        return self.pred.view(self.B, self.cfg.chunk, self.cfg.action_dim)

    def _attn(self, i: int, fwd: bool, dout=None):
        B, T, D, Ka, Kt, H = self.B, self.cfg.chunk, self.D, self.Ka, self.Kt, self.H
        qkv = self.QKVx[i].view(B, T, 3 * D)
        ka = self.KV_adp[i].view(B, Ka, 2 * D)
        kt = self.KV_task[i].view(B, Kt, 2 * D)
        args = (qkv[:, :, :D], qkv[:, :, D:2 * D], qkv[:, :, 2 * D:], ka[:, :, :D], ka[:, :, D:], kt[:, :, :D], kt[:, :, D:])
        gate = self.P.view("gate")[i]
        out = self.AOx[i].view(B, T, D)
        if fwd:
            ops.head_attn_fwd(*args, gate, H, self.ref_softmax, out=out, probs=self.probs[i])
        else:
            g = self.dQKVx[i].view(B, T, 3 * D)
            ga = self.dKV_adp[i].view(B, Ka, 2 * D)
            gt = self.dKV_task[i].view(B, Kt, 2 * D)
            ops.head_attn_bwd(dout.view(B, T, D), out, *args, gate, self.probs[i], self.dgate[i:i + 1], g[:, :, :D], g[:, :, D:2 * D],
                              g[:, :, 2 * D:], ga[:, :, :D], ga[:, :, D:], gt[:, :, :D], gt[:, :, D:], H,
                              rope=self.rope_tab if self.pro else None)

    def backward(self, dpred: torch.Tensor, dHS: torch.Tensor, row0: int = 0):
        self.prep_backward(self.pos1, self.Np, self.B, self.S, row0)
        self.bwd_begin(dpred, row0)
        for i in range(self.nb - 1, -1, -1):
            self.bwd_layer(i, dHS)
        self.bwd_end()

    def prep_backward(self, pos1: torch.Tensor, Np: int, B: int, S: int, row0: int, pos0=None, cnt0=None):
        self._alloc(B, Np)
        g = self.guard if pos0 is not None else None
        ops.head_index_prep(pos1, pos0 if pos0 is not None else pos1, cnt0 if cnt0 is not None else pos1, self._idx_scratch,
                            self.row_idx_live_ka, g, B, S, Np, row0)
        self._prep_key = (B, S, Np, row0)

    def bwd_begin(self, dpred: torch.Tensor, row0: int = 0):
        cfg, P, nb = self.cfg, self.P, self.nb
        R, Da = self.R, cfg.action_dim
        self.row0 = row0
        assert self._prep_key == (self.B, self.S, self.Np, row0), "prep_backward() first"
        self.refresh_transposes()
        ops.zero_(self.acc32)
        dp = dpred.reshape(R, Da)
        ops.zero_(self.dpad)
        ops.copy2d(dp, self.dpad, R, Da, Da, 64)
        ops.colsum_(dp, self.b_f32["fc2_b"])
        self._dw(self.dpad, self.xf_ln, out=self.dfc2)
        ops.copy2d(self.dfc2, P.g("fc2_w"), Da, self.D, self.D, self.D)
        d_ln2 = ops.gemm_nt(self.dpad, self.fc2T)
        self.dx = ops.layernorm_bwd(d_ln2, self.X[nb], P.view("ln2_w"), self.st2, self.ln2_dw, self.ln2_db)

    def bwd_layer(self, i: int, dHS: torch.Tensor):
        P, D = self.P, self.D
        B, S, Kt, Ka = self.B, self.S, self.Kt, self.Ka
        dff = self.dFF[i]
        ops.relu_bwd(self.dx, self.X[i + 1], out=dff)
        d_ln = ops.gemm_nt(dff, self.T["w_ffn"][i])
        do2 = self.dO2[i]
        ops.layernorm_bwd(d_ln, self.O2[i], P.view("ln_w")[i], self.stats[i], self.ln_dw[i], self.ln_db[i], out=do2)
        d_ao = ops.gemm_nt(do2, self.T["w_o"][i])
        self._attn(i, fwd=False, dout=d_ao)
        self.dx = ops.gemm_nt(self.dQKVx[i], self.T["w_x"][i], residual=do2)
        ops.gemm_nt(self.dKV_adp[i], self._kv("adp", i)[2], out=self.dh_adp[i])
        ops.scatter_add_rows(self.dh_adp[i], self.row_idx_live_ka.view(-1), dHS[i + 1].view(-1, D))
        if self.row0 == 0:
            ops.gemm_nt(self.dKV_task[i], self._kv("task", i)[2], out=dHS[i + 1].view(B * S, D)[:B * Kt], c_group=(Kt, S * D))

    def bwd_end(self):
        cfg, P, D, nb = self.cfg, self.P, self.D, self.nb
        B, Ka = self.B, self.Ka
        G = P.g
        dy1 = ops.relu_bwd(self.dx, self.X[0])
        ops.colsum_(dy1, self.b_f32["fc1_b"])
        self._dw(dy1, self.x_ln, out=G("fc1_w"))
        d_xln = ops.gemm_nt(dy1, self._t(P.view("fc1_w")))
        ops.layernorm_bwd(d_xln, self.x_in, P.view("ln1_w"), self.st1, self.ln1_dw, self.ln1_db, want_dx=False)
        ops.colsum_(self.dh_adp.view(nb, B, Ka, D)[:, :, NUM_TOKENS].transpose(0, 1), self.d_pf32)
        d_pf = ops.cast_f32_bf16(self.d_pf32)
        ops.colsum_(d_pf, self.b_f32["p_fc2_b"])
        self._dw(d_pf, self.pp_act, out=G("p_fc2_w"))
        d_act = ops.gemm_nt(d_pf, self.T["p_fc2_w"])
        d_pre = ops.gelu_bwd(d_act, self.pp_pre)
        ops.colsum_(d_pre, self.b_f32["p_fc1_b"])
        self._dw(d_pre, self.pr_in, out=self.dpfc1)
        ops.copy2d(self.dpfc1, G("p_fc1_w"), D, cfg.proprio_dim, 64, cfg.proprio_dim)
        Kt, S = self.Kt, self.S
        h_adp = self.h_adp.view(nb, B * Ka, D)
        if self.h_task_c is None:
            h_task, tg = self.HSref[1:nb + 1, 0, :Kt], (Kt, S * D)
        else:
            for i in range(nb):
                ops.copy_rows3d(self.HSref[i + 1], self.h_task_c[i], B, Kt, D, S * D, D, Kt * D, D)
            h_task, tg = self.h_task_c, None
        ops.gemm_tn(self.dQKVx, self.X[:nb], out=G("w_x"))
        ops.gemm_tn(self.dO2, self.AOx, out=G("w_o"))
        ops.gemm_tn(self.dFF, self.LNo, out=G("w_ffn"))
        ops.colsum_(self.dQKVx, self.b_f32["b_x"]); ops.colsum_(self.dO2, self.b_f32["b_o"]); ops.colsum_(self.dFF, self.b_f32["b_ffn"])
        if self.pro:
            ops.gemm_tn(self.dKV_adp, h_adp, out=G("w_adp"))
            ops.gemm_tn(self.dKV_task, h_task, out=G("w_task"), rows=B * Kt, b_group=tg)
            ops.colsum_(self.dKV_adp, self.b_f32["b_adp"]); ops.colsum_(self.dKV_task, self.b_f32["b_task"])
        else:
            gkv = G("w_x")[:, self.D:]
            ops.gemm_tn(self.dKV_adp, h_adp, out=gkv, accumulate=True)
            ops.gemm_tn(self.dKV_task, h_task, out=gkv, accumulate=True, rows=B * Kt, b_group=tg)
            bkv = self.b_f32["b_x"][:, self.D:]
            ops.colsum_(self.dKV_adp, bkv); ops.colsum_(self.dKV_task, bkv)
        for k, t in self.b_f32.items():
            ops.cast_f32_bf16(t, out=G(k))
        ops.cast_f32_bf16(self.ln_dw, out=G("ln_w")); ops.cast_f32_bf16(self.ln_db, out=G("ln_b"))
        ops.cast_f32_bf16(self.ln1_dw, out=G("ln1_w")); ops.cast_f32_bf16(self.ln1_db, out=G("ln1_b"))
        ops.cast_f32_bf16(self.ln2_dw, out=G("ln2_w")); ops.cast_f32_bf16(self.ln2_db, out=G("ln2_b"))
        ops.copy2d(self.dgate, G("gate"), nb, 1, 1, 8)

    def _t(self, w2d):
        return ops.transpose(w2d.contiguous())

    def _dw(self, dy, x, out=None):
        return ops.gemm_tn(dy, x, out=out, split=0)


class Workspace:
    FIELDS = ("feats", "patches", "_vis_bufs", "B", "S", "Np", "qidx0", "pos0", "cnt0", "pos1", "cnt1", "_pred_out", "_dHS")

    def __init__(self, llm: Optional[dict] = None, head: Optional[dict] = None, fields: Optional[dict] = None):
        self.llm, self.head, self.fields = llm, head, fields or dict.fromkeys(self.FIELDS)


class VLAEngine(schedule.StepControls):

    def __init__(self, cfg: VLACfg, weights: Dict, device="cuda"):
        self.cfg, self.device = cfg, device
        self.vits = [ViT(c, sd, device, j) for j, (c, sd) in enumerate(zip(cfg.vit, weights["vit"]))]
        self.llm = LLM(cfg.llm, weights["llm"], device)
        self.head = Head(cfg, device)
        self.head.load_state_dicts(weights["head"], weights["proprio"], weights.get("action_queries"))
        g = lambda k: weights["proj"][k].to(device=device, dtype=BF16).contiguous()
        self.proj = {k: g(k) for k in weights["proj"]}
        self.step_count = 0
        self._ws = None
        self.bind_workspace(Workspace())
        self.full_llm_backward = bool(int(os.environ.get("VLA_FULL_LLM_BWD", "0")))
        self._row0 = None
        self.reducer = None
        self._init_step_controls(copy_flat, ops.add_)
        self.executed_steps = 0
        self.n_act = min(cfg.llm.n_layers, cfg.num_blocks)
        self.fp8_frozen = False
        self.side = None
        self._vis_bufs = {}
        self._val_pred = None
        self._predict_graphs, self._val_graphs = {}, None
        self._generate_sets = {}
        self._timeline = None
        self._graphs = self._g_vis = self._vis_ev = self._px_copied = self._pending_lr = self._reduced = None
        if os.environ.get("VLA_FP8_FROZEN"):
            self.enable_fp8_frozen()

    def enable_fp8_frozen(self):
        for v in self.vits:
            v.enable_fp8()
        self.llm.enable_fp8()
        self.fp8_frozen = True

    def _grad_buffers(self):
        return [self.head.P.grad]

    def _state_buffers(self):
        return [("head", self.head.P)]

    @property
    def frozen_row0(self) -> Optional[int]:
        return self._row0

    def _set_clip(self, clip):
        self.flush()
        self._clip = clip
        if clip is not None:
            clip.begin(self._clip_ranges())
            self._clip_events = (torch.cuda.Event(), torch.cuda.Event())

    def _clip_ranges(self):
        g, aq_off = self.head.P.grad, self.head.P.offsets["action_queries"][0]
        return [(g, 0, aq_off), (g, aq_off, self.head.P.numel)]

    def workspace(self, head: bool = True) -> Workspace:
        self._ws = Workspace(self.llm.buffer_set(), self.head.buffer_set() if head else None, {k: getattr(self, k) for k in Workspace.FIELDS})
        return self._ws

    def bind_workspace(self, ws: Workspace):
        if ws is self._ws and ws.llm is self.llm._bound and (ws.head is None or ws.head is self.head._bound):
            return
        self.llm.unbind() if ws.llm is None else self.llm.bind_buffer_set(ws.llm)
        if ws.head is not None:
            self.head.bind_buffer_set(ws.head)
        for k, v in ws.fields.items():
            setattr(self, k, v)
        self._ws = ws

# ... 241 lines not shown
        return self._dHS

    def _prep_backward(self, actions, row0: Optional[int] = None):
        frozen = row0 is not None
        self._row0_used = row0 = row0 if frozen else self.live_row0()
        self._dhs(row0)
        self.head.prep_backward(self.pos1, self.Np, self.B, self.S, row0, self.pos0, self.cnt0)
        self._guard = self.head.guard if frozen and row0 else None
        self._actions_bf = self._to_bf16(actions)

    def _turn_around(self, pred, gscale: float) -> torch.Tensor:
        loss3, dpred = ops.l1_loss(pred, self._actions_bf, True, gscale)
        if self._guard is not None:
            ops.add_scalar_f32_(loss3, self._guard)
        self.head.bwd_begin(dpred, self._row0_used)
        return loss3

    def _query_grad(self):
        dq = ops.action_query_grad(self.llm.bwd_result().contiguous(), self.pos0, self.Np, self._row0_used)
        ops.cast_f32_bf16(dq, out=self.head.P.g("action_queries"))

    def loss_and_backward(self, pred, actions, gscale: float = 1.0, exchange: bool = True):
        llm, head = self.llm, self.head
        exchange = exchange and self.reducer is not None
        self._prep_backward(actions)
        loss3 = self._turn_around(pred, gscale)
        for i in range(head.nb - 1, -1, -1):
            head.bwd_layer(i, self._dHS)
        head.bwd_end()
        aq_off = head.P.offsets["action_queries"][0]
        if exchange:
            self.reducer.reduce_async(head.P.grad, 0, aq_off)
        llm.backward(self._dHS, self.B, self.S, self._row0_used, n_run=self.n_act)
        self._query_grad()
        if exchange:
            self.reducer.reduce_async(head.P.grad, aq_off, None)
        return loss3

    def optimizer_step(self, lr: float, beta1=0.9, beta2=0.999, eps=1e-8, wd=0.01):
        self._apply_update(lr, beta1, beta2, eps, wd, two_stream=False, join=False)

    def train_step(self, batch, lr: float, noise=None):
        self.executed_steps += 1
        pred = self.forward(batch, noise, for_training=True)
        loss3 = self.loss_and_backward(pred, batch["actions"], 1.0 / self.ga, exchange=self.ga == 1)
        if self._accum.fold():
            if self.ga > 1 and self.reducer is not None:
                self.reducer.reduce_async(self.head.P.grad, 0, None)
            self.optimizer_step(lr)
        return loss3

    def _ensure_streams(self):
        if self.side is None:
            self.side = torch.cuda.Stream()
            self._cap_main = torch.cuda.Stream()
            self.vis_stream = torch.cuda.Stream()
            self._vstreams = [self.vis_stream] + [torch.cuda.Stream() for _ in range(max(0, len(self.vits) - 1))]

    def _segments(self, batch, noise):
        llm, head = self.llm, self.head
        n = self.n_act
        fch = turnaround_chunks(n, 4, [2, 1, 1], 1)
        if os.environ.get("VLA_FWD_CHUNKS"):
            fch = chunks(n, [int(x) for x in os.environ["VLA_FWD_CHUNKS"].split(",")])

        def llm_fwd(c, lo, hi):
            if c == 0:
                mm = self._embed(batch)
                self._prep_backward(batch["actions"], self._row0)
                llm.fwd_begin(self.B, self.S, mm, self._row0_used)
            llm.fwd_layers(lo, hi)

        def turn_around():
            self._loss3 = self._turn_around(head.fwd_end(), 1.0 / self.ga)

        def llm_bwd(k, lo, hi):
            if k == 0:
                llm.bwd_begin(self._dHS, self._row0_used, n)
            for i in range(hi - 1, lo - 1, -1):
                llm.bwd_layer(i, self._dHS)
            if k == len(fch) - 1:
                self._query_grad()

        return (schedule.pipeline_forward(head, fch, llm_fwd, lambda: (llm.HS, self.pos1, batch["proprio"], self.Np, noise), turn_around,
                                          refresh=True)
                + schedule.pipeline_backward(head, fch, llm_bwd, lambda: self._dHS)
                + [Segment("H", head.bwd_end, None, ("end", 0))])

    def _stream_of(self, name: str, main):
        return main if name == "M" else self.side if name == "H" else self._vstreams[int(name[1:])]

    def _cap_stream(self, name: str):
        return self._cap_main if name == "M" else self._stream_of(name, None)

    def _fwd_bwd(self, batch, noise, vision: bool = True):
        self.executed_steps += 1
        if vision:
            self._vision(batch)
        torch.cuda.current_stream().wait_event(schedule.run(self._segments(batch, noise), self._stream_of)[("end", 0)])
        return self._loss3

    def capture(self, batch: Dict[str, torch.Tensor], noise: Optional[torch.Tensor] = None, warmup: int = 2,
                conservative_rows: bool = False, row0: Optional[int] = None):
        self._ensure_streams()
        self._static_batch, self._static_noise = batch, noise
        self._row0 = None
        self._vision_and_embed(batch)
        self._row0 = self.live_row0()
        if conservative_rows and not self.full_llm_backward:
            self._row0 = min(self._row0, (self.cfg.n_patches + 1) // 32 * 32)
        if row0 is not None:
            assert 0 <= int(row0) < self.S and int(row0) % 32 == 0, f"row0 {row0}: a multiple of 32 inside the sequence"
            self._row0 = int(row0)
        for _ in range(warmup):
            self.head.dirty = True
            self._fwd_bwd(batch, noise)
        torch.cuda.synchronize()
        self.head.dirty = True
        self._next_px = batch["pixel_values"].clone()
        self._px_stage = batch["pixel_values"].clone()
        self._g_vis = capture_graph(lambda: self._vision(dict(batch, pixel_values=self._px_stage)), torch.cuda.graph_pool_handle(),
                                    self.vis_stream)
        self._vis_ev = None
        self._segs = self._segments(batch, noise)
        self._graphs = schedule.capture(self._segs, {}, self._cap_stream)
        torch.cuda.synchronize()
        self._step_ws = self.workspace()
        self._pending_lr = None
        m_fwd = [k for k, sg in enumerate(self._segs) if sg.stream == "M" and sg.signal is not None and sg.signal[0] == "f"]
        self._vis_after = m_fwd[min(len(m_fwd) - 1, max(0, int(os.environ.get("VLA_VIS_AFTER", len(m_fwd) - 4))))]
        assert self._segs[self._vis_after].signal is not None
        self._launch_vision()

    def stage_next_pixels(self, pixel_values: torch.Tensor):
        if self._px_copied is not None:
            torch.cuda.current_stream().wait_event(self._px_copied)
        self._next_px.copy_(pixel_values)

    def _launch_vision(self, after_event=None):
        V, cur = self.vis_stream, torch.cuda.current_stream()
        if after_event is not None:
            V.wait_event(after_event)
        else:
            V.wait_stream(cur)
        tl = self._timeline
        with torch.cuda.stream(V):
            if tl is not None:
                t0 = torch.cuda.Event(enable_timing=True)
                t0.record(V)
            copy_flat(self._px_stage, self._next_px)
            self._px_copied = torch.cuda.Event()
            self._px_copied.record(V)
            self._g_vis.replay()
            self._vis_ev = torch.cuda.Event(enable_timing=tl is not None)
            self._vis_ev.record(V)
            if tl is not None:
                tl.append(("V", -1, t0, self._vis_ev))

    def train_step_pipelined(self, batch, lr: float, noise=None):
        self._ensure_streams()
        loss3 = self._fwd_bwd(batch, noise)
        if self.reducer is not None:
            self.reducer.reduce_async(self.head.P.grad, 0, None)
        self.optimizer_step(lr)
        return loss3

    def train_step_graphed(self, lr: float):
        cur = torch.cuda.current_stream()
# ... 108 lines not shown
```

### vla_adapter_amd/native.py

```python
from __future__ import annotations

import ctypes as C
import os
from typing import NamedTuple

_HERE = os.path.dirname(os.path.abspath(__file__))
LIB_PATH = (os.environ.get("VLA_NATIVE_LIB") or None) or os.path.join(_HERE, "libvla_native.so")

ACT_NONE, ACT_GELU, ACT_RELU, ACT_GELU_TANH, ACT_SWIGLU, ACT_SWIGLU_BWD = 0, 1, 2, 3, 4, 5
KERNEL_NT_SKINNY, KERNEL_NT_64x128_S6, KERNEL_NT_128x128_S4, KERNEL_NT_128x128, KERNEL_NT_128x64, KERNEL_NT_256 = 0, 8, 9, 10, 11, 12
KERNEL_TN_128, KERNEL_TN_256 = 16, 17
ABI_VERSION = 8


class NativeLibraryMissing(ImportError):
    pass


class GemmDesc(C.Structure):
    _fields_ = [("A", C.c_void_p), ("B", C.c_void_p), ("C", C.c_void_p), ("bias", C.c_void_p), ("R", C.c_void_p),
                ("C2", C.c_void_p),
                ("M", C.c_int), ("N", C.c_int), ("K", C.c_int), ("lda", C.c_int), ("ldb", C.c_int), ("ldc", C.c_int),
                ("ldr", C.c_int), ("ldc2", C.c_int), ("res_mod", C.c_int), ("act", C.c_int), ("batch", C.c_int),
                ("sA", C.c_longlong), ("sB", C.c_longlong), ("sC", C.c_longlong), ("sR", C.c_longlong),
# ... 110 lines not shown
        "vla_dropout_bwd_add_bf16": ([_P, _P, _P, _L, C.c_int, _L, _L, C.c_float, C.c_ulonglong, _P], _I),
        "vla_inc_i32": ([_P, _P], _I),
        "vla_quant_fp8_rows": ([_P, _P, _P, _P, _I, _I, _I, _I], _I),
        "vla_rmsnorm_fwd_q8": ([_P, _P, _P, _P, _P, _P, _P, _I, _I, _I, _F], _I),
        "vla_layernorm_fwd_q8": ([_P, _P, _P, _P, _P, _P, _P, _P, _I, _I, _I, _I, _I, _F], _I),
        "vla_head_index_prep": ([_P, _P, _P, _P, _P, _P, _P, _I, _I, _I, _I], _I),
        "vla_add_scalar_f32": ([_P, _P, _P, _I], _I),
        "vla_head_attn_fwd": ([_P, C.POINTER(HeadAttnDesc)], _I),
        "vla_head_attn_bwd": ([_P, C.POINTER(HeadAttnDesc)], _I),
        "vla_l1_loss": ([_P, _P, _P, _P, _P, _I, _I, _I, _F], _I),
        "vla_adamw_bf16": ([_P, _P, _P, _P, _P, _L, _D, _D, _D, _D, _D, _I, _I, _F], _I),
        "vla_adamw_clipped_bf16": ([_P, _P, _P, _P, _P, _L, _D, _D, _D, _D, _D, _I, _I, _F, _P], _I),
        "vla_grad_sumsq_slots": ([_L], _L),
        "vla_grad_sumsq": ([_P, _P, _L, _I, _F, _P], _I),
        "vla_grad_norm_finalise": ([_P, _P, _L, _F, _P], _I),
        "vla_normalize_bounds": ([_P, _P, _P, _L, _I, _P, _P, _P, _P], _I),
        "vla_collate_tokens": ([_P, _P, _P, _L, _P, _P, _P, _P, _P, _I, _I, _I, _I, _F, _F, _L, _L, _L, _I, C.c_ulonglong, _L, _L], _I),
    }),
    Family("serve", "vla_serve.h", {
        "vla_serve_tokens": ([_P, _P, _P, _L, _P, _P, _P, _P, _P, _I, _I, _I, _L, _L, _L, _L, _L], _I),
        "vla_normalize_proprio_serve": ([_P, _P, _I, _P, _L, _I, _P, _P, _P], _I),
        "vla_unnormalize_actions": ([_P, _P, _P, _I, _I, _I, _I, _I, _P, _P, _P, _P], _I),
        "vla_serve_gather_hidden": ([_P, _P, _P, _P, _I, _I, _I, _I, _I, _L, _I], _I),
    }),
    Family("episodes", "vla_episodes.h", {
        "vla_episode_sample": ([_P, _P, _P, _P, _I, C.c_ulonglong, _L, _L, _L, _I, _I, _P, _P, _P], _I),
        "vla_episode_gather": ([_P, _P, _P, _P, _P, _P, _P, _P, _P, _P, _P, _P, _P, _P, _I, _I, _L, _L, _I, _I, _I, _L, _I], _I),
    }),
    Family("mixture", "vla_mixture.h", {
        "vla_mixture_sample": ([_P, _P, _P, _P, _P, _P, _I, _I, C.c_ulonglong, _L, _L, _L, _I, _I, _P, _P, _P, _P], _I),
        "vla_normalize_bounds_rows": ([_P, _P, _P, _L, _I, _I, _P, _I, _P, _P, _P, _P], _I),
    }),
    Family("heldout", "vla_heldout.h", {
        "vla_heldout_sweep": ([_P, _P, _P, _P, _P, _I, _I, _L, _L, _L, _L, _I, _I, _P, _P, _P, _P, _P], _I),
        "vla_heldout_l1_accumulate": ([_P, _P, _P, _P, _P, _I, _I, _I, _I, _P, _P], _I),
    }),
    Family("digest", "vla_digest.h", {
        "vla_state_digest_slots": ([], _I),
        "vla_state_digest": ([_P, _P, _L, C.c_ulonglong, _P, _L, _P], _I),
        "vla_token_ce_metrics_ordered": ([_P, _P, _L, _P, _P, _I, _I, _P, _P, _P, _L, _I, _P], _I),
    }),
    Family("jpeg", "vla_jpeg.h", {
        "vla_jpeg_workspace_bytes": ([_L, _I, _I, _I], _L),
        "vla_jpeg_decode_rows": ([_P, _P, _L, _P, _P, _L, _P, _P, _I, _P, _I, _P, _I, _L, _P, _P, _I, _I, _I, _I, _I, _I, _I, _P, _L, _P, _L, _P], _I),
    }),
    Family("jpeg_index", "vla_jpeg_index.h", {
        "vla_jpeg_index_build": ([_P, _P, _L, _P, _P, _L, _P, _P, _I, _P, _I, _L, _I, _I, _I, _I, _P, _L, _L, _I, _P, _P, _L, _P], _I),
        "vla_jpeg_decode_rows_at": ([_P, _P, _L, _P, _P, _P, _L, _P, _P, _I, _P, _I, _P, _I, _L, _P, _P, _I, _I, _I, _I, _I, _I, _I, _P, _L, _P, _L, _P], _I),
    }),
    Family("policy_image", "vla_policy_image.h", {
        "vla_policy_image_workspace_bytes": ([_L, _I, _I, _I, _I, _I], _L),
        "vla_policy_jpeg_round_trip": ([_P, _P, _L, _L, _I, _I, _P, _P, _L, _P, _L], _I),
        "vla_policy_lanczos3_resize": ([_P, _P, _L, _L, _I, _I, _I, _I, _P, _P, _I, _P, _P, _I, _P, _L, _P], _I),
    }),
)
PROTOS = {name: sig for fam in FAMILIES for name, sig in fam.protos.items()}
assert len(PROTOS) == sum(len(fam.protos) for fam in FAMILIES), "an entry point belongs to one header"

LATER_FAMILIES = (
    Family("jpeg_encode", "vla_jpeg_encode.h", {
        "vla_jpeg_encode_workspace_bytes": ([_L, _I, _I, _I], _L),
        "vla_jpeg_encode_plan": ([_P, _P, _L, _L, _I, _I, _P, _I, _P, _L, _P], _I),
        "vla_jpeg_encode_write": ([_P, _L, _I, _I, _P, _I, _P, _L, _P, _P, _L], _I),
    }),
)
LATER_PROTOS = {name: sig for fam in LATER_FAMILIES for name, sig in fam.protos.items()}
assert len(LATER_PROTOS) == sum(len(fam.protos) for fam in LATER_FAMILIES) and not set(LATER_PROTOS) & set(PROTOS), "an entry point belongs to one header"


ADDED_FAMILIES = (
    Family("decode", "vla_decode.h", {
        "vla_decode_prompt": ([_P, _P, _P, _L, _P, _P, _P, _P, _P, _I, _I, _I, _L], _I),
        "vla_decode_rope_append": ([_P, _P, _P, _P, _P, _P, _P, _I, _I, _I, _I, _I, _I, _L, _I], _I),
        "vla_decode_attn": ([_P, _P, _P, _P, _P, _P, _I, _I, _I, _I, _I, _I, _I, _L, _I, _F], _I),
        "vla_decode_argmax_slabs": ([_I], _I),
        "vla_decode_lm_head_argmax": ([_P, _P, _I, _P, _I, _I, _I, _I, _P, _P, _P, _P, _L, _P, _I, _P, _P, _P, _P, _I, _I, _P, _I], _I),
    }),
)
ADDED_PROTOS = {name: sig for fam in ADDED_FAMILIES for name, sig in fam.protos.items()}
assert len(ADDED_PROTOS) == sum(len(fam.protos) for fam in ADDED_FAMILIES) and not set(ADDED_PROTOS) & (set(PROTOS) | set(LATER_PROTOS)), \
    "an entry point belongs to one header"
ALL_FAMILIES = FAMILIES + LATER_FAMILIES + ADDED_FAMILIES


def family(key: str) -> Family:
    return next(fam for fam in ALL_FAMILIES if fam.key == key)


_lib = None


def load():
    global _lib
    if _lib is not None:
        return _lib
    if not os.path.exists(LIB_PATH):
        raise NativeLibraryMissing(
            f"{LIB_PATH} not found: build it with `python -c 'import __graft_entry__ as g; g.build()'` "
            f"(or `make -C {os.path.join(_HERE, 'csrc')}`).  There is no CPU/PyTorch fallback.")
    lib = C.CDLL(LIB_PATH)
    for name, (args, res) in [sig for fam in ALL_FAMILIES for sig in fam.protos.items()]:
        fn = getattr(lib, name, None)
        if fn is None:
            raise NativeLibraryMissing(f"{LIB_PATH} does not export {name}: it was built from an older source tree, rebuild (make -C csrc)")
        fn.argtypes, fn.restype = args, res
    lib.vla_last_error.argtypes, lib.vla_last_error.restype = [], C.c_char_p
    if lib.vla_version() != ABI_VERSION:
        raise NativeLibraryMissing(f"{LIB_PATH} speaks ABI {lib.vla_version()}, this binding ABI {ABI_VERSION}: rebuild (make -C csrc)")
    for which, st in enumerate((GemmDesc, AttnDesc, HeadAttnDesc, GemmTnDesc)):
        if lib.vla_desc_size(which) != C.sizeof(st):
            raise NativeLibraryMissing(f"{LIB_PATH}: sizeof({st.__name__}) is {lib.vla_desc_size(which)} in the library, {C.sizeof(st)} in the binding")
    _lib = lib
    return lib


class NativeError(RuntimeError):
    pass


def check(rc: int, what: str = ""):
    if rc != 0:
        msg = load().vla_last_error().decode(errors="replace")
        raise NativeError(f"libvla_native: {what} failed with code {rc}: {msg}")
```

### vla_adapter_amd/ops.py

```python
from __future__ import annotations

import ctypes as C
import math
from typing import Optional, Tuple

import torch

from . import native as N
from .native import ACT_GELU, ACT_GELU_TANH, ACT_NONE, ACT_RELU, ACT_SWIGLU, ACT_SWIGLU_BWD
from .scratch import ARENA

BF16 = torch.bfloat16


def _lib():
    return N.load()


def _st():
    return C.c_void_p(torch.cuda.current_stream().cuda_stream)


def _p(t: Optional[torch.Tensor]):
    return None if t is None else C.c_void_p(t.data_ptr())


def _chk_bf16(*ts):
    for t in ts:
        if t is not None:
            assert t.is_cuda and t.dtype == BF16, f"expected CUDA bf16 tensor, got {t.device} {t.dtype}"


def gemm_nt(a: torch.Tensor, b: torch.Tensor, *, bias=None, residual=None, res_mod: int = 0, act: int = ACT_NONE,
            out: Optional[torch.Tensor] = None, out2: Optional[torch.Tensor] = None, alpha: float = 1.0,
            want_pre: bool = True, a_group=None, c_group=None, r_group=None, rope=None, c_live=None,
            split_k: Optional[int] = None, bias_post_round: bool = False, fp8=None, ext=None, query_256: bool = False,
            query_plan: bool = False):
    if fp8 is not None:
        assert a.dtype == torch.uint8 and b.dtype == torch.uint8 and a.dim() == 2 and split_k in (None, 0, 1)
        _chk_bf16(bias, residual, out, out2)
        split_k = 0
    else:
        _chk_bf16(a, b, bias, residual, out, out2)
    assert a.stride(-1) == 1 and b.stride(-1) == 1
    batched = a.dim() == 3
    if batched:
        nb, M, K = a.shape
        sA = a.stride(0)
        sB = b.stride(0) if b.dim() == 3 else 0
        Nn = b.shape[-2]
    else:
        nb, (M, K), sA, sB, Nn = 1, a.shape, 0, 0, b.shape[0]
    assert b.shape[-1] == K, f"K mismatch {a.shape} x {b.shape}"
    d = N.GemmDesc()
    d.A, d.B = a.data_ptr(), b.data_ptr()
    d.M, d.N, d.K, d.lda, d.ldb, d.batch = M, Nn, K, a.stride(-2), b.stride(-2), nb
    d.sA, d.sB, d.act, d.alpha, d.res_mod = sA, sB, act, alpha, res_mod
    shape = (nb, M, Nn) if batched else (M, Nn)
    if act == ACT_SWIGLU:
        if out is None and want_pre:
            out = torch.empty(shape, device=a.device, dtype=BF16)
        hshape = shape[:-1] + (Nn // 2,)
        if out2 is None:
            out2 = torch.empty(hshape, device=a.device, dtype=BF16)
        assert out2.shape == hshape and out2.stride(-1) == 1
        d.C2, d.ldc2, d.sC2 = out2.data_ptr(), out2.stride(-2), (out2.stride(0) if batched else 0)
    elif out is None:
        out = torch.empty(shape, device=a.device, dtype=BF16)
    if out is not None:
        assert tuple(out.shape) == tuple(shape) and out.stride(-1) == 1, f"out shape {out.shape} != {shape}"
        d.C, d.ldc, d.sC = out.data_ptr(), out.stride(-2), (out.stride(0) if batched else 0)
    if bias is not None:
        assert bias.shape[-1] == Nn and bias.stride(-1) == 1
        d.bias = bias.data_ptr()
        d.sBias = bias.stride(0) if bias.dim() == 2 else 0
    if residual is not None:
        assert residual.stride(-1) == 1 and residual.shape[-1] == Nn
        assert res_mod > 0 or r_group is not None or tuple(residual.shape) == tuple(shape)
        d.R, d.ldr = residual.data_ptr(), residual.stride(-2)
        d.sR = residual.stride(0) if (batched and residual.dim() == 3) else 0
    if a_group is not None:
        d.a_group, d.a_group_stride = a_group
    if c_group is not None:
        d.c_group, d.c_group_stride = c_group
    if r_group is not None:
        d.r_group, d.r_group_stride = r_group
    if c_live is not None:
        d.c_live_mod, d.c_live_from = c_live
    if rope is not None:
        mode, cos_t, sin_t, T, dh, ncols = rope
        assert cos_t.dtype == torch.float32 and cos_t.is_contiguous() and sin_t.is_contiguous() and cos_t.shape[0] >= T
        assert cos_t.shape[1] == (dh // 2 if mode == 1 else dh)
        d.rope_mode, d.rope_T, d.rope_dh, d.rope_cols = mode, T, dh, ncols
        d.rope_cos, d.rope_sin = cos_t.data_ptr(), sin_t.data_ptr()
    if fp8 is not None:
        sa, sb = fp8
        assert sa.dtype == torch.float32 and sb.dtype == torch.float32 and sa.numel() == M and sb.numel() == Nn and sa.is_contiguous() and sb.is_contiguous()
        d.fp8, d.a_scale, d.b_scale = 1, sa.data_ptr(), sb.data_ptr()
    if ext is not None:
        a2, b2 = ext
        _chk_bf16(a2, b2)
        assert not batched and a2.dim() == 2 and b2.dim() == 2 and a2.shape[0] == M and b2.shape[0] == Nn and a2.shape[1] == b2.shape[1]
        assert a2.stride(1) == 1 and b2.stride(1) == 1 and a2.shape[1] % 64 == 0 and split_k in (None, 0, 1)
        d.A2, d.B2, d.K2, d.lda2, d.ldb2 = a2.data_ptr(), b2.data_ptr(), a2.shape[1], a2.stride(0), b2.stride(0)
        split_k = 0
    if bias_post_round:
        assert bias is not None
        d.bias_post_round = 1
    if split_k is None and not batched and K >= 2048:
        split_k = _nt_plan(d)[1]
    if split_k and split_k > 1:
        d.split_k, d.ws = split_k, _scratch_f32(split_k * M * Nn, a.device).data_ptr()
    if query_plan or query_256:
        plan = _nt_plan(d)
        return plan if query_plan else plan[0] == N.KERNEL_NT_256
    N.check(_lib().vla_gemm_bf16_nt(_st(), C.byref(d)), "gemm_bf16_nt")
    if act == ACT_SWIGLU:
        return out, out2
    return out


def _nt_plan(d) -> Tuple[int, int]:
    split = C.c_int(0)
    kernel = _lib().vla_gemm_nt_plan(C.byref(d), -1, 0, C.byref(split))
    N.check(min(kernel, 0), "gemm_nt_plan")
    return kernel, split.value


def gemm_plan(a: torch.Tensor, b: torch.Tensor, **kw) -> Tuple[int, int]:
    return gemm_nt(a, b, query_plan=True, **kw)


class latency_hint:

    def __enter__(self):
        self.prev = _lib().vla_gemm_latency_hint(1)
        return self

    def __exit__(self, *exc):
        _lib().vla_gemm_latency_hint(self.prev)
        return False


def _scratch_f32(numel: int, device) -> torch.Tensor:
    return ARENA.get(4 * numel, device).view(torch.float32)


def gemm_swiglu_bwd(d: torch.Tensor, w_downT: torch.Tensor, gu: torch.Tensor, out: Optional[torch.Tensor] = None,
                    gu_group=None, ext=None, fp8=None, query_plan: bool = False):
    if fp8 is not None:
        assert ext is not None and d.dtype == torch.uint8 and w_downT.dtype == torch.uint8
        _chk_bf16(gu, out)
    else:
        _chk_bf16(d, w_downT, gu, out)
    M, K = d.shape
    I = w_downT.shape[0]
    assert gu.shape[-1] == 2 * I and gu.stride(-1) == 1 and w_downT.shape[1] == K
    assert gu_group is not None or gu.shape[0] == M
    if out is None:
        out = torch.empty(M, 2 * I, device=d.device, dtype=BF16)
    assert out.shape == (M, 2 * I)
    desc = N.GemmDesc()
    desc.A, desc.B, desc.C, desc.R = d.data_ptr(), w_downT.data_ptr(), out.data_ptr(), gu.data_ptr()
    desc.M, desc.N, desc.K, desc.lda, desc.ldb, desc.ldc, desc.ldr, desc.batch = M, I, K, d.stride(0), w_downT.stride(0), out.stride(0), gu.stride(0), 1
    desc.act, desc.alpha = ACT_SWIGLU_BWD, 1.0
    if gu_group is not None:
        desc.r_group, desc.r_group_stride = gu_group
    if ext is not None:
        a2, b2 = ext
        _chk_bf16(a2, b2)
        assert a2.shape == (M, b2.shape[1]) and b2.shape[0] == I and a2.stride(1) == 1 and b2.stride(1) == 1 and a2.shape[1] % 64 == 0
        desc.A2, desc.B2, desc.K2, desc.lda2, desc.ldb2 = a2.data_ptr(), b2.data_ptr(), a2.shape[1], a2.stride(0), b2.stride(0)
    if fp8 is not None:
        sa, sb = fp8
        assert sa.dtype == torch.float32 and sb.dtype == torch.float32 and sa.numel() == M and sb.numel() == I and sa.is_contiguous() and sb.is_contiguous()
        desc.fp8, desc.a_scale, desc.b_scale = 1, sa.data_ptr(), sb.data_ptr()
    if query_plan:
        return _nt_plan(desc)
    N.check(_lib().vla_gemm_bf16_nt(_st(), C.byref(desc)), "gemm_bf16_nt(swiglu_bwd)")
    return out


def gemm_tn(a: torch.Tensor, b: torch.Tensor, *, out: Optional[torch.Tensor] = None, alpha: float = 1.0, accumulate: bool = False,
            a_group=None, b_group=None, a_cols=None, rows: Optional[int] = None, split: Optional[int] = None) -> torch.Tensor:
    _chk_bf16(a, b, out)
    assert a.stride(-1) == 1 and b.stride(-1) == 1 and a.dim() == b.dim()
    batched = a.dim() == 3
    nb = a.shape[0] if batched else 1
    M = rows if rows is not None else a.shape[-2]
    assert rows is not None or b.shape[-2] == M
    N1, N2 = a.shape[-1], b.shape[-1]
    d = N.GemmTnDesc()
    a_ptr = a.data_ptr()
    if a_cols is not None:
        N1, cg, cgs, off = a_cols
        assert cg % 8 == 0 and cgs % 8 == 0 and off % 8 == 0
        d.a_col_group, d.a_col_group_stride = cg, cgs
        a_ptr += off * 2
    shape = (nb, N1, N2) if batched else (N1, N2)
    if out is None:
        assert not accumulate
        out = torch.empty(shape, device=a.device, dtype=BF16)
    assert tuple(out.shape) == shape and out.stride(-1) == 1, f"out shape {tuple(out.shape)} != {shape}"
    d.A, d.B, d.C = a_ptr, b.data_ptr(), out.data_ptr()
    d.M, d.N1, d.N2, d.lda, d.ldb, d.ldc, d.batch = M, N1, N2, a.stride(-2), b.stride(-2), out.stride(-2), nb
    d.sA, d.sB, d.sC = (a.stride(0), b.stride(0), out.stride(0)) if batched else (0, 0, 0)
    d.alpha = alpha
    if accumulate:
        d.R, d.ldr, d.sR = out.data_ptr(), out.stride(-2), d.sC
    if a_group is not None:
        d.a_group, d.a_group_stride = a_group
    if b_group is not None:
        d.b_group, d.b_group_stride = b_group
# ... 1051 lines not shown
```

### vla_adapter_amd/trainers.py

```python
from __future__ import annotations

import contextlib
import math
import os
from typing import Dict, List, Optional, Tuple

import torch

from . import engine as E
from . import ops, schedule
from .schedule import Segment, capture_graph, chunks, turnaround_chunks
from .ops import BF16

rup = E.rup


class LoraLinear:

    def __init__(self, name: str, n_out: int, k_in: int, projs, r: int, k_real: Optional[int] = None, n_real: Optional[int] = None):
        self.name, self.n_out, self.k_in, self.projs, self.r = name, n_out, k_in, projs, r
        self.k_real, self.n_real = k_real or k_in, n_real or n_out
        self.rp = rup(r, 64)
        self.Rr = self.rp * len(projs)

# ... 234 lines not shown
                cs(dh_, a("b2"))
            dm = self._lin_bwd(k + "fc2", dh_, st["Mact"][i], b["w2T"], out=st["G_pre"][i])
            ops.gelu_bwd(dm, st["Mpre"][i], out=dm)
            dpre = dm
            if tv:
                cs(dpre, a("b1"))
            dh2 = self._lin_bwd(k + "fc1", dpre, st["H2"][i], b["w1T"], out=st["g_d"])
            ops.layernorm_bwd(dh2, st["Xm"][i], b["n2w"], st["S2"][i], a("n2w"), a("n2b"), out=dxm)
            ops.add_(dxm, dx)
            da_ = ops.layerscale_bwd(dxm, st["PA"][i] if tv else None, b["ls1"], a("ls1"), out=st["G_proj"][i]) if ls else dxm
            if tv:
                cs(da_, a("bproj"))
            da = self._lin_bwd(k + "proj", da_, st["A"][i], b["wprojT"], out=st["g_d"])
            qkv = st["QKV"][i].view(Bv, T, 3 * d)
            g_mid = st["G_qkv"][i]
            dqkv = g_mid.view(Bv, T, 3 * d)
            ops.attn_bwd(da.view(Bv, T, d), qkv[:, :, :d], qkv[:, :, d:2 * d], qkv[:, :, 2 * d:], st["A"][i].view(Bv, T, d), st["LSE"][i],
                         vc.heads, vc.heads, dh, False, None, dq=dqkv[:, :, :d], dk=dqkv[:, :, d:2 * d], dv=dqkv[:, :, 2 * d:])
            if tv:
                cs(g_mid, a("bqkv"))
            dh1 = self._lin_bwd(k + "qkv", g_mid, st["H1"][i], b["wqkvT"], out=st["g_d"])
            if i == 0 and not tv:
                return
            dxi = self._vit_grad_slots(j, i - 1)[0] if i > 0 else st["dxa"]
            ops.layernorm_bwd(dh1, st["X"][i], b["n1w"], st["S1"][i], a("n1w"), a("n1b"), out=dxi)
            ops.add_(dxi, dxm)
            if tap is not None:
                tap["d_in"] = dxi.clone()

    def _vit_bwd_end(self, j: int):
        v, st, cfg = self.vits[j], self.V[j], self.cfg
        vc = v.cfg
        npi, T, d = vc.n_patches, vc.n_patches + vc.n_prefix, vc.d
        Bv = self.eng.B * cfg.n_img
        dx = st["dxa"]
        if vc.n_prefix:
            dpe = st["pe"]
            ops.copy_rows3d(dx.view(Bv, T, d)[0, vc.n_prefix:], dpe, Bv, npi, d, T * d, d, npi * d, d)
            ops.colsum_(dx.view(Bv, T * d)[:, :vc.n_prefix * d], self.A(f"vit{j}.prefix"))
        else:
            dpe = dx
        self._defer_tn(dpe, st["cols"], self.G(f"vit{j}.wpe"))
        ops.colsum_(dpe, self.A(f"vit{j}.bpe"))
        ops.colsum_(dpe.view(Bv, npi * d), self.A(f"vit{j}.pos"))

    def _segments(self, batch, noise, gscale: float = 1.0, actions=None):
        if self.objective == "token_ce":
            return self._segments_ce(batch, gscale)
        eng, cfg, llm, head = self.eng, self.cfg, self.llm, self.head
        el, na = self.exchange_layers, self.n_active
        lch = chunks(na, [el]) if os.environ.get("VLA_UNIFORM_CHUNKS") else turnaround_chunks(na, el, [2, 1, 1], el)
        segs = []
        add, grads = self._builders(segs)
        side = self.vstream is not None

        def f_pre():
            eng._vision_begin(batch)
            self._alloc(eng.B, eng.S)
            self._begin_forward()

        def f_front():
            if not side:
                f_pre()
            for j in range(1 if side else len(self.vits)):
                self._vit_forward(j, batch["pixel_values"])

        def f_front2():
            self._proj_forward()
            self._mm = eng._embed(batch)
            self._batch = batch
            llm.fwd_begin(eng.B, eng.S, self._mm, 0, lin=self)
            if not self._evaluating:
                self._begin_backward()
                self._dHS = eng._dhs(0)
        if side:
            add("M", f_pre, None, ("pre", 0))
            add("V", lambda: self._vit_forward(1, batch["pixel_values"]), ("pre", 0), ("vf", 1))
        add("M", f_front, None, None)
        add("M", f_front2, ("vf", 1) if side else None, ("front", 0))

        def fwd_end():
            self._pred = head.fwd_end()
        segs += schedule.pipeline_forward(head, lch, lambda c, lo, hi: llm.fwd_layers(lo, hi),
                                          lambda: (llm.HS, eng.pos1, batch["proprio"], eng.Np, noise), fwd_end, refresh=True)
        self._n_forward = len(segs)

        def h_loss():
            tgt = eng._to_bf16(batch["actions"] if actions is None else actions)
            self._loss3, dpred = ops.l1_loss(self._pred, tgt, True, gscale)
            head.prep_backward(eng.pos1, eng.Np, eng.B, eng.S, 0)
            head.bwd_begin(dpred, 0)
        add("H", h_loss, None, None)
        aq_off = head.P.offsets["action_queries"][0]
        segs += schedule.pipeline_backward(head, lch, lambda k, lo, hi: self._llm_bwd_layers(lo, hi), lambda: self._dHS,
                                           lambda k, lo, hi: self._grads(("m", k), ("g", k), self._ranges("llm", lo, hi - 1)))
        add("H", head.bwd_end, None, ("hend", 0), [(head.P.grad, 0, aq_off)])
        add("M", self._mid_backward, None, ("mid", 0))
        grads(("mid", 0), ("gmid", 0), [(head.P.grad, aq_off, head.P.numel)] + self._ranges("embed") + self._ranges("proj"))
        self._vit_bwd_segments(add, grads, side)
        if self.trains_vectors:
            add("M", self._end_backward, [sg.signal for sg in segs if sg.stream == "G"], ("end", 0), self._ranges("tail"))
        return segs

    def _grads(self, after, signal, ranges) -> Segment:
        if self.gstream is not None:
            return Segment("G", self._flush_work, after, signal, ranges)
        return Segment("M", None, None, signal, ranges)

    def _builders(self, segs):
        def add(st, fn, wait=None, signal=None, ranges=None):
            segs.append(Segment(st, fn, wait, signal, ranges))
        return add, lambda after, signal, ranges: segs.append(self._grads(after, signal, ranges))

    def _vit_bwd_segments(self, add, grads, side: bool):
        vsegs = []
        for j in range(len(self.vits)):
            for q, (lo, hi) in enumerate(reversed(self._vit_chunks(j))):
                def v_bwd(j=j, lo=lo, hi=hi, first=(q == 0)):
                    if first:
                        self._vit_bwd_begin(j)
                    self._vit_bwd_blocks(j, lo, hi)
                    if lo == 0 and self.trains_vectors:
                        self._vit_bwd_end(j)
                vsegs.append((j, q, lo, hi, v_bwd))
        if side:
            a, b = [x for x in vsegs if x[0] == 0], [x for x in vsegs if x[0] == 1]
            vsegs = [x for pair in zip(a, b) for x in pair] + a[len(b):] + b[len(a):]
        for j, q, lo, hi, v_bwd in vsegs:
            on_side = side and j == 1
            add("V" if on_side else "M", v_bwd, ("mid", 0) if on_side and q == 0 else None, ("v", j, q))
            grads(("v", j, q), ("gv", j, q), self._ranges("vit", lo, hi - 1, j))

    def _segments_ce(self, batch, gscale: float = 1.0):
        eng, cfg, llm = self.eng, self.cfg, self.llm
        n, D, V = cfg.llm.n_layers, cfg.llm.d, cfg.llm.vocab
        assert getattr(llm, "lm_head", None) is None, "token-CE training: tied lm_head only (Qwen2.5-0.5B / 1.5B tie_word_embeddings)"
        lch = chunks(n, [self.exchange_layers])
        segs = []
        add, grads = self._builders(segs)

        def f_front():
            eng._vision_begin(batch)
            self._alloc(eng.B, eng.S)
            self._begin_forward()
            for j in range(len(self.vits)):
                self._vit_forward(j, batch["pixel_values"])
            self._proj_forward()
            self._mm = eng._embed(batch, action_queries=False)
            self._batch = batch
            llm.fwd_begin(eng.B, eng.S, self._mm, 0, lin=self)
            self._begin_backward()
            self._dHS = eng._dhs(0)
        add("M", f_front, None, ("front", 0))
        for c, (lo, hi) in enumerate(lch):
            add("M", lambda lo=lo, hi=hi: llm.fwd_layers(lo, hi), None, ("f", c))
        self._n_forward = len(segs)

        def f_ce():
            B, S, Np = eng.B, eng.S, eng.Np
            Lm = S - Np - 1
            if self._ce_key != (B, S):
                e = lambda *sh, dt=BF16: torch.empty(*sh, device=self.dev, dtype=dt)
                self.ce_h, self.ce_dh, self.ce_logits = e(B * Lm, D), e(B * Lm, D), e(B * Lm, V)
                self.ce_out = torch.zeros(2, device=self.dev, dtype=torch.float32)
                self.ce_cls = torch.empty(B, Lm, device=self.dev, dtype=torch.uint8)
                self.ce_counters = torch.zeros(6, device=self.dev, dtype=torch.int64)
                self.ce_metrics = torch.empty(4, device=self.dev, dtype=torch.float32)
# ... 826 lines not shown
```

Measured before the change: 1358.

## Add NN GEMM path for action-head backward and batch f32 grad casts

Adds an NN variant of the bf16 GEMM kernel that reads the weight operand row-major and transposes it in LDS with ds_read_tr16 reads. The action head's backward dx GEMMs now use it on the live weights, so the per-step transposed weight copies (refresh_transposes) and their buffers go away. It also replaces the many per-tensor f32→bf16 gradient casts with a single segmented cast kernel. The cost is that every NN GEMM is forced onto the fixed 128x128 tile with no planner choice, which may suit small or skinny shapes worse than the NT path did.

Measured after the change: 1357 (median of 2 runs). Within noise of the previous version (-0.1%).

```diff
diff --git a/include/vla_head_dx.h b/include/vla_head_dx.h
--- /dev/null
+++ b/include/vla_head_dx.h
@@ -0,0 +1,17 @@
+#ifndef VLA_HEAD_DX_H
+#define VLA_HEAD_DX_H
+
+#include "vla_native.h"
+
+#ifdef __cplusplus
+extern "C" {
+#endif
+
+int vla_gemm_bf16_nn(void* stream, const vla_gemm_desc* desc );
+
+int vla_cast_f32_bf16_segments(void* stream, const float* x, void* y, const long long* table , int count);
+
+#ifdef __cplusplus
+}
+#endif
+#endif
diff --git a/vla_adapter_amd/csrc/common.h b/vla_adapter_amd/csrc/common.h
--- a/vla_adapter_amd/csrc/common.h
+++ b/vla_adapter_amd/csrc/common.h
@@ -145,6 +145,10 @@
                : "=&s"(keep) : "v"(voff), "s"(base), "s"(dst) : "memory");
 }
 
+__device__ __forceinline__ bf16x4 tr_read(const char* p) {
+  return __builtin_amdgcn_ds_read_tr16_b64_v4i16((__attribute__((address_space(3))) bf16x4*)p);
+}
+
 __device__ __forceinline__ v8i_f8 cat8(bf16x8 lo, bf16x8 hi) {
   typedef float f32x8 __attribute__((ext_vector_type(8)));
   const f32x4 l = __builtin_bit_cast(f32x4, lo), h = __builtin_bit_cast(f32x4, hi);
diff --git a/vla_adapter_amd/csrc/elementwise.hip b/vla_adapter_amd/csrc/elementwise.hip
--- a/vla_adapter_amd/csrc/elementwise.hip
+++ b/vla_adapter_amd/csrc/elementwise.hip
@@ -1,5 +1,6 @@
 #include "gemm_epilogue.h"
 #include "argmax_order.h"
+#include "../../include/vla_head_dx.h"
 #include <type_traits>
 
 namespace {
@@ -224,6 +225,16 @@
 
 __global__ void cast_f32_bf16_kernel(const float* __restrict__ x, bf16_t* __restrict__ y, long long n) {
   for (long long i = (long long)blockIdx.x * blockDim.x + threadIdx.x; i < n; i += (long long)gridDim.x * blockDim.x) y[i] = f2bf(x[i]);
+}
+constexpr int CAST_SEG_MAX = 32, CAST_SEG_CHUNK = 1024;
+struct CastSegs { long long src[CAST_SEG_MAX], dst[CAST_SEG_MAX], n[CAST_SEG_MAX]; int start[CAST_SEG_MAX + 1]; int count; };
+__global__ void cast_f32_bf16_segments_kernel(const float* __restrict__ x, bf16_t* __restrict__ y, CastSegs S) {
+  int si = 0;
+  while (si + 1 < S.count && (int)blockIdx.x >= S.start[si + 1]) ++si;
+  const long long i0 = (long long)((int)blockIdx.x - S.start[si]) * CAST_SEG_CHUNK, i1 = min(S.n[si], i0 + CAST_SEG_CHUNK);
+  const float* xs = x + S.src[si];
+  bf16_t* ys = y + S.dst[si];
+  for (long long i = i0 + threadIdx.x; i < i1; i += blockDim.x) ys[i] = f2bf(xs[i]);
 }
 __global__ void cast_bf16_f32_kernel(const bf16_t* __restrict__ x, float* __restrict__ y, long long n) {
   for (long long i = (long long)blockIdx.x * blockDim.x + threadIdx.x; i < n; i += (long long)gridDim.x * blockDim.x) y[i] = bf2f(x[i]);
@@ -599,6 +610,23 @@
   VLA_REQUIRE(x && y && n > 0, "cast: bad args");
   hipLaunchKernelGGL(cast_f32_bf16_kernel, GRID1D(n, 256), dim3(256), 0, (hipStream_t)stream, x, (bf16_t*)y, n);
   VLA_CHECK_LAUNCH("cast_f32_bf16");
+  return VLA_OK;
+}
+extern "C" int vla_cast_f32_bf16_segments(void* stream, const float* x, void* y, const long long* table, int count) {
+  VLA_REQUIRE(x && y && table && count > 0 && count <= CAST_SEG_MAX, "cast_segments: 1 .. 32 segments");
+  CastSegs S;
+  long long chunks = 0;
+  for (int i = 0; i < count; ++i) {
+    VLA_REQUIRE(table[3 * i] >= 0 && table[3 * i + 1] >= 0 && table[3 * i + 2] > 0, "cast_segments: offsets >= 0, n > 0");
+    S.src[i] = table[3 * i]; S.dst[i] = table[3 * i + 1]; S.n[i] = table[3 * i + 2];
+    S.start[i] = (int)chunks;
+    chunks += (S.n[i] + CAST_SEG_CHUNK - 1) / CAST_SEG_CHUNK;
+    VLA_REQUIRE(chunks < (1LL << 30), "cast_segments: too many elements for one launch");
+  }
+  S.start[count] = (int)chunks;
+  S.count = count;
+  hipLaunchKernelGGL(cast_f32_bf16_segments_kernel, dim3((unsigned)chunks), dim3(256), 0, (hipStream_t)stream, x, (bf16_t*)y, S);
+  VLA_CHECK_LAUNCH("cast_f32_bf16_segments");
   return VLA_OK;
 }
 extern "C" int vla_cast_bf16_f32(void* stream, const void* x, float* y, long long n) {
diff --git a/vla_adapter_amd/csrc/gemm.hip b/vla_adapter_amd/csrc/gemm.hip
--- a/vla_adapter_amd/csrc/gemm.hip
+++ b/vla_adapter_amd/csrc/gemm.hip
@@ -1,6 +1,7 @@
 #include <algorithm>
 #include "gemm_epilogue.h"
 #include "gemm_params.h"
+#include "../../include/vla_head_dx.h"
 
 namespace {
 
@@ -35,10 +36,11 @@
   static_assert(PIECES % NW == 0, "pieces must divide evenly over the waves");
 };
 
-template <int BM, int BN, int STAGES, int ROPE, int WN = 2, bool F8 = false, bool EXT = false>
+template <int BM, int BN, int STAGES, int ROPE, int WN = 2, bool F8 = false, bool EXT = false, bool NN = false>
 __global__ __launch_bounds__((BM / 64) * 64 * WN) __attribute__((amdgpu_waves_per_eu((F8 && EXT) ? 4 : 1)))
 void gemm_nt_kernel(GemmP p) {
   using C = Cfg<BM, BN, STAGES, WN>;
+  static_assert(!NN || (BN == 128 && ROPE == 0 && !F8 && !EXT), "the NN form: 128-column tiles of a plain bf16 product");
   constexpr int EB = F8 ? 1 : 2;
   extern __shared__ __attribute__((aligned(16))) char smem[];
   const int tid = threadIdx.x, lane = tid & 63;
@@ -64,6 +66,11 @@
     if (pc < BM / 8) {
       const int ra = min(m0 + pc * 8 + (lane >> 3), p.M - 1);
       pp[i] = Ab + grouped_row(ra, p.gA, p.sgA, p.lda) * EB + kc;
+    } else if constexpr (NN) {
+      const int r = 4 * (pc - BM / 8) + (lane >> 4);
+      const int f = ((r & 3) << 2) | ((r >> 2) & 3);
+      const int col = min(n0 + (((lane & 15) ^ f) << 3), p.N - 8);
+      pp[i] = Bb + ((long long)r * p.ldb + col) * 2;
     } else {
       const int rb = min(n0 + (pc - BM / 8) * 8 + (lane >> 3), p.N - 1);
       pp[i] = Bb + (long long)rb * p.ldb * EB + kc;
@@ -84,6 +91,10 @@
     if (EXT && t >= nt1) {
 #pragma unroll
       for (int i = 0; i < C::PPW; ++i) glds16(pp2[i] + (t - nt1) * 128, base + i * 1024);
+    } else if constexpr (NN) {
+      const long long bstep = (long long)p.ldb * (BK * 2);
+#pragma unroll
+      for (int i = 0; i < C::PPW; ++i) glds16(pp[i] + (wid * C::PPW + i < BM / 8 ? t * 128LL : t * bstep), base + i * 1024);
     } else {
 #pragma unroll
       for (int i = 0; i < C::PPW; ++i) glds16(pp[i] + t * 128, base + i * 1024);
@@ -102,6 +113,17 @@
   for (int s = 0; s < 2; ++s) {
     foff[s] = frow * 128 + (((F8 ? 2 * (lane >> 4) + s : 4 * s + (lane >> 4)) ^ (lane & 7)) << 4);
     foff2[s] = frow * 128 + (((4 * s + (lane >> 4)) ^ (lane & 7)) << 4);
+  }
+
+  int ftr[NN ? C::NT : 1][2];
+  if constexpr (NN) {
+    const int kq = lane >> 4, qq = (lane >> 2) & 3, tp = lane & 3;
+#pragma unroll
+    for (int e = 0; e < 2; ++e) {
+      const int row = 8 * kq + qq + 4 * e, f = (qq << 2) | ((2 * kq + e) & 3);
+#pragma unroll
+      for (int i = 0; i < C::NT; ++i) ftr[i][e] = 256 * row + ((((wc * C::WTN + i * 16) >> 3) + (tp >> 1)) ^ f) * 16 + 8 * (tp & 1);
+    }
   }
 
   const int wm0 = m0 + wr * 64, wn0 = n0 + wc * C::WTN;
@@ -154,7 +176,14 @@
     bf16x8 fm[2][4], fn[2][C::NT];                                                                                                   \
     _Pragma("unroll") for (int s = 0; s < 2; ++s) {                                                                                  \
       _Pragma("unroll") for (int i = 0; i < 4; ++i) fm[s][i] = *reinterpret_cast<const bf16x8*>(sa + i * 16 * 128 + FO[s]);          \
-      _Pragma("unroll") for (int i = 0; i < C::NT; ++i) fn[s][i] = *reinterpret_cast<const bf16x8*>(sb + cbase(i) * 128 + FO[s]);    \
+      if constexpr (NN) {                                                                                                            \
+        _Pragma("unroll") for (int i = 0; i < C::NT; ++i) {                                                                          \
+          const bf16x4 lo = tr_read(sb + s * 8192 + ftr[i][0]), hi = tr_read(sb + s * 8192 + ftr[i][1]);                             \
+          fn[s][i] = bf16x8{lo[0], lo[1], lo[2], lo[3], hi[0], hi[1], hi[2], hi[3]};                                                 \
+        }                                                                                                                            \
+      } else {                                                                                                                       \
+        _Pragma("unroll") for (int i = 0; i < C::NT; ++i) fn[s][i] = *reinterpret_cast<const bf16x8*>(sb + cbase(i) * 128 + FO[s]);  \
+      }                                                                                                                              \
     }                                                                                                                                \
     if constexpr (F8T) {                                                                                                             \
       _Pragma("unroll") for (int ni = 0; ni < C::NT; ++ni)                                                                           \
@@ -457,14 +486,14 @@
   }
 }
 
-template <int BM, int BN, int STAGES, int ROPE, int WN = 2, bool F8 = false, bool EXT = false>
+template <int BM, int BN, int STAGES, int ROPE, int WN = 2, bool F8 = false, bool EXT = false, bool NN = false>
 int launch(const GemmP& p0, int nb, hipStream_t st) {
   using C = Cfg<BM, BN, STAGES, WN>;
-  if (int rc = vla_lds_limit<gemm_nt_kernel<BM, BN, STAGES, ROPE, WN, F8, EXT>>(C::LDS_BYTES, "gemm_nt_kernel")) return rc;
+  if (int rc = vla_lds_limit<gemm_nt_kernel<BM, BN, STAGES, ROPE, WN, F8, EXT, NN>>(C::LDS_BYTES, "gemm_nt_kernel")) return rc;
   GemmP p = p0;
   p.tiles_n = (p.N + BN - 1) / BN;
   p.ntiles = ((p.M + BM - 1) / BM) * p.tiles_n;
-  hipLaunchKernelGGL((gemm_nt_kernel<BM, BN, STAGES, ROPE, WN, F8, EXT>), dim3(p.ntiles, 1, nb), dim3(C::NTHREADS), C::LDS_BYTES, st, p);
+  hipLaunchKernelGGL((gemm_nt_kernel<BM, BN, STAGES, ROPE, WN, F8, EXT, NN>), dim3(p.ntiles, 1, nb), dim3(C::NTHREADS), C::LDS_BYTES, st, p);
   return VLA_OK;
 }
 
@@ -630,7 +659,9 @@
   return pl.kernel;
 }
 
-extern "C" int vla_gemm_bf16_nt(void* stream, const vla_gemm_desc* d) {
+namespace {
+
+int gemm_run(void* stream, const vla_gemm_desc* d, const bool nn) {
   VLA_REQUIRE(d && d->A && d->B, "gemm: null operand");
   VLA_REQUIRE(d->M > 0 && d->N > 0 && d->K > 0 && d->batch > 0, "gemm: empty problem");
   VLA_REQUIRE(d->K % BK == 0, "gemm: K must be a multiple of 64 (pad the operands)");
@@ -686,9 +717,14 @@
                                        "gemm: fused rotate_half RoPE needs head dim 64, or 128 with N and rope_cols multiples of 128");
   }
 
+  if (nn)
+    VLA_REQUIRE(d->C && d->N >= 8 && d->N % 8 == 0 && d->ldb >= d->N && d->act == VLA_ACT_NONE && !d->fp8 && d->K2 == 0 && d->rope_mode == 0 && d->a_group == 0 &&
+                    d->r_group == 0 && d->res_mod == 0 && d->c_live_mod == 0 && d->bias_post_round == 0,
+                "gemm_nn: bf16 operands, N % 8 == 0, and a plain / bias / residual epilogue with batch strides, c_group or split_k");
   const NtOverrides ov = nt_overrides();
   const int ncu = vla_num_cus();
-  const NtPlan pl = plan_nt(d, g_latency_hint > 0, ncu, ov);
+  NtPlan pl = plan_nt(d, g_latency_hint > 0, ncu, ov);
+  if (nn) pl.kernel = VLA_KERNEL_NT_128x128;
 
   GemmP p;
   p.A = (const bf16_t*)d->A; p.B = (const bf16_t*)d->B; p.C = (bf16_t*)d->C;
@@ -709,6 +745,7 @@
     p.K = (kt + pl.split - 1) / pl.split * BK;
     p.Ktot = d->K;
     p.sA = p.sB = p.K;
+    if (nn) p.sB = (long long)p.K * d->ldb;
     p.bias = nullptr; p.R = nullptr;
   }
   p.rope_mode = d->rope_mode; p.rope_T = d->rope_T; p.rope_dh = d->rope_dh; p.rope_cols = d->rope_cols;
@@ -720,7 +757,8 @@
   const int nb = pl.split > 1 ? pl.split : d->batch;
   const int rope = d->act == VLA_ACT_SWIGLU_BWD ? 3 : d->rope_mode;
   int rc;
-  if (pl.kernel < VLA_KERNEL_NT_SKINNY + SKINNY_TILES) rc = vla_gemm_skinny_launch(p, pl.kernel - VLA_KERNEL_NT_SKINNY, st);
+  if (nn) rc = launch<128, 128, 2, 0, 4, false, false, true>(p, nb, st);
+  else if (pl.kernel < VLA_KERNEL_NT_SKINNY + SKINNY_TILES) rc = vla_gemm_skinny_launch(p, pl.kernel - VLA_KERNEL_NT_SKINNY, st);
   else if (pl.kernel == VLA_KERNEL_NT_256)
     rc = vla_gemm256_launch(p, d->act == VLA_ACT_SWIGLU ? 1 : d->act == VLA_ACT_SWIGLU_BWD ? 2 : 0, d->batch, ov.grid_set ? ov.grid : ncu, st);
   else if (d->K2 > 0 && d->fp8)
@@ -739,3 +777,9 @@
   if (pl.split > 1) return splitk_finalize(d, pl.split, st);
   return VLA_OK;
 }
+
+}
+
+extern "C" int vla_gemm_bf16_nt(void* stream, const vla_gemm_desc* d) { return gemm_run(stream, d, false); }
+
+extern "C" int vla_gemm_bf16_nn(void* stream, const vla_gemm_desc* d) { return gemm_run(stream, d, true); }
diff --git a/vla_adapter_amd/csrc/gemm_tn.hip b/vla_adapter_amd/csrc/gemm_tn.hip
--- a/vla_adapter_amd/csrc/gemm_tn.hip
+++ b/vla_adapter_amd/csrc/gemm_tn.hip
@@ -18,10 +18,6 @@
   int cgA, cgsA;
   int tiles_n2, ntiles, split, mslice;
 };
-
-__device__ __forceinline__ bf16x4 tr_read(const char* p) {
-  return __builtin_amdgcn_ds_read_tr16_b64_v4i16((__attribute__((address_space(3))) bf16x4*)p);
-}
 
 __device__ __forceinline__ void tn_tile(const TnP& p, const int swz, const int bz, char* smem) {
   const int tid = threadIdx.x, lane = tid & 63;
diff --git a/vla_adapter_amd/engine.py b/vla_adapter_amd/engine.py
--- a/vla_adapter_amd/engine.py
+++ b/vla_adapter_amd/engine.py
@@ -595,10 +595,7 @@
         self.P = FlatParams(spec, device)
         self.film = {}
         z = lambda *s: torch.zeros(*s, device=device, dtype=BF16)
-        self.T = dict(w_x=z(nb, D, 3 * D), w_o=z(nb, D, D), w_ffn=z(nb, D, D), p_fc2_w=z(D, D))
-        if cfg.pro:
-            self.T.update(w_adp=z(nb, D, 2 * D), w_task=z(nb, D, 2 * D))
-        self.fc2T = z(D, 64)
+        self.fc2_pad = z(64, D)
         self.pfc1_pad = z(D, 64)
         self.dirty = True
         self.rope_tab = None
@@ -618,8 +615,8 @@
     def _kv(self, which: str, i: int):
         D = self.D
         if self.pro:
-            return self.P.view("w_" + which)[i], self.P.view("b_" + which)[i], self.T["w_" + which][i]
-        return self.P.view("w_x")[i, D:], self.P.view("b_x")[i, D:], self.T["w_x"][i][:, D:]
+            return self.P.view("w_" + which)[i], self.P.view("b_" + which)[i]
+        return self.P.view("w_x")[i, D:], self.P.view("b_x")[i, D:]
 
     def named_views(self, buf=None) -> Dict[str, torch.Tensor]:
         P, D, out = self.P, self.D, {}
@@ -660,29 +657,11 @@
         sd.update(self.film)
         return sd
 
-    @property
-    def dirty(self) -> bool:
-        return self._stale_fwd or self._stale_bwd
-
-    @dirty.setter
-    def dirty(self, v: bool):
-        self._stale_fwd = self._stale_bwd = bool(v)
-
     def refresh_forward_operands(self):
-        if self._stale_fwd:
+        if self.dirty:
             pd = self.cfg.proprio_dim
             ops.copy2d(self.P.view("p_fc1_w"), self.pfc1_pad, self.D, pd, pd, self.pfc1_pad.stride(0))
-            self._stale_fwd = False
-
-    def refresh_transposes(self):
-        if not self._stale_bwd:
-            return
-        P = self.P
-        for k in (("w_x", "w_adp", "w_task", "w_o", "w_ffn") if self.pro else ("w_x", "w_o", "w_ffn")):
-            ops.transpose(P.view(k), out=self.T[k])
-        ops.transpose(P.view("p_fc2_w"), out=self.T["p_fc2_w"])
-        ops.transpose(P.view("fc2_w"), out=self.fc2T)
-        self._stale_bwd = False
+            self.dirty = False
 
     def build_buffer_set(self, B: int, Kt: int) -> dict:
         D, nb, T, dev = self.D, self.nb, self.cfg.chunk, self.device
@@ -753,9 +732,9 @@
         hs2 = HS[i + 1].view(B * S, D)
         ops.gather_rows(hs2, self.row_idx_ka.view(-1), self.h_adp[i].view(B * Ka, D))
         fuse = self.pro and D % 64 == 0 and not os.environ.get("VLA_NO_KV_ROPE_FUSE")
-        wa, ba, _ = self._kv("adp", i)
+        wa, ba = self._kv("adp", i)
         ops.gemm_nt(self.h_adp[i].view(B * Ka, D), wa, bias=ba, out=self.KV_adp[i], rope=(2, rc, rs_, Ka, dh, D) if fuse else None)
-        wt, bt, _ = self._kv("task", i)
+        wt, bt = self._kv("task", i)
         ops.gemm_nt(hs2[:B * Kt], wt, bias=bt, out=self.KV_task[i], a_group=(Kt, S * D), bias_post_round=B > 1,
                     rope=(2, rc, rs_, Kt, dh, D) if fuse else None)
         x = self.X[i]
@@ -814,7 +793,6 @@
         R, Da = self.R, cfg.action_dim
         self.row0 = row0
         assert self._prep_key == (self.B, self.S, self.Np, row0), "prep_backward() first"
-        self.refresh_transposes()
         ops.zero_(self.acc32)
         dp = dpred.reshape(R, Da)
         ops.zero_(self.dpad)
@@ -822,7 +800,8 @@
         ops.colsum_(dp, self.b_f32["fc2_b"])
         self._dw(self.dpad, self.xf_ln, out=self.dfc2)
         ops.copy2d(self.dfc2, P.g("fc2_w"), Da, self.D, self.D, self.D)
-        d_ln2 = ops.gemm_nt(self.dpad, self.fc2T)
+        ops.copy2d(P.view("fc2_w"), self.fc2_pad, Da, self.D, self.D, self.D)
+        d_ln2 = ops.gemm_nn(self.dpad, self.fc2_pad)
         self.dx = ops.layernorm_bwd(d_ln2, self.X[nb], P.view("ln2_w"), self.st2, self.ln2_dw, self.ln2_db)
 
     def bwd_layer(self, i: int, dHS: torch.Tensor):
@@ -830,16 +809,16 @@
         B, S, Kt, Ka = self.B, self.S, self.Kt, self.Ka
         dff = self.dFF[i]
         ops.relu_bwd(self.dx, self.X[i + 1], out=dff)
-        d_ln = ops.gemm_nt(dff, self.T["w_ffn"][i])
+        d_ln = ops.gemm_nn(dff, P.view("w_ffn")[i])
         do2 = self.dO2[i]
         ops.layernorm_bwd(d_ln, self.O2[i], P.view("ln_w")[i], self.stats[i], self.ln_dw[i], self.ln_db[i], out=do2)
-        d_ao = ops.gemm_nt(do2, self.T["w_o"][i])
+        d_ao = ops.gemm_nn(do2, P.view("w_o")[i])
         self._attn(i, fwd=False, dout=d_ao)
-        self.dx = ops.gemm_nt(self.dQKVx[i], self.T["w_x"][i], residual=do2)
-        ops.gemm_nt(self.dKV_adp[i], self._kv("adp", i)[2], out=self.dh_adp[i])
+        self.dx = ops.gemm_nn(self.dQKVx[i], P.view("w_x")[i], residual=do2)
+        ops.gemm_nn(self.dKV_adp[i], self._kv("adp", i)[0], out=self.dh_adp[i])
         ops.scatter_add_rows(self.dh_adp[i], self.row_idx_live_ka.view(-1), dHS[i + 1].view(-1, D))
         if self.row0 == 0:
-            ops.gemm_nt(self.dKV_task[i], self._kv("task", i)[2], out=dHS[i + 1].view(B * S, D)[:B * Kt], c_group=(Kt, S * D))
+            ops.gemm_nn(self.dKV_task[i], self._kv("task", i)[0], out=dHS[i + 1].view(B * S, D)[:B * Kt], c_group=(Kt, S * D))
 
     def bwd_end(self):
         cfg, P, D, nb = self.cfg, self.P, self.D, self.nb
@@ -848,13 +827,13 @@
         dy1 = ops.relu_bwd(self.dx, self.X[0])
         ops.colsum_(dy1, self.b_f32["fc1_b"])
         self._dw(dy1, self.x_ln, out=G("fc1_w"))
-        d_xln = ops.gemm_nt(dy1, self._t(P.view("fc1_w")))
+        d_xln = ops.gemm_nn(dy1, P.view("fc1_w"))
         ops.layernorm_bwd(d_xln, self.x_in, P.view("ln1_w"), self.st1, self.ln1_dw, self.ln1_db, want_dx=False)
         ops.colsum_(self.dh_adp.view(nb, B, Ka, D)[:, :, NUM_TOKENS].transpose(0, 1), self.d_pf32)
         d_pf = ops.cast_f32_bf16(self.d_pf32)
         ops.colsum_(d_pf, self.b_f32["p_fc2_b"])
         self._dw(d_pf, self.pp_act, out=G("p_fc2_w"))
-        d_act = ops.gemm_nt(d_pf, self.T["p_fc2_w"])
+        d_act = ops.gemm_nn(d_pf, P.view("p_fc2_w"))
         d_pre = ops.gelu_bwd(d_act, self.pp_pre)
         ops.colsum_(d_pre, self.b_f32["p_fc1_b"])
         self._dw(d_pre, self.pr_in, out=self.dpfc1)
@@ -881,15 +860,10 @@
             ops.gemm_tn(self.dKV_task, h_task, out=gkv, accumulate=True, rows=B * Kt, b_group=tg)
             bkv = self.b_f32["b_x"][:, self.D:]
             ops.colsum_(self.dKV_adp, bkv); ops.colsum_(self.dKV_task, bkv)
-        for k, t in self.b_f32.items():
-            ops.cast_f32_bf16(t, out=G(k))
-        ops.cast_f32_bf16(self.ln_dw, out=G("ln_w")); ops.cast_f32_bf16(self.ln_db, out=G("ln_b"))
-        ops.cast_f32_bf16(self.ln1_dw, out=G("ln1_w")); ops.cast_f32_bf16(self.ln1_db, out=G("ln1_b"))
-        ops.cast_f32_bf16(self.ln2_dw, out=G("ln2_w")); ops.cast_f32_bf16(self.ln2_db, out=G("ln2_b"))
+        accs = dict(self.b_f32, ln_w=self.ln_dw, ln_b=self.ln_db, ln1_w=self.ln1_dw, ln1_b=self.ln1_db, ln2_w=self.ln2_dw, ln2_b=self.ln2_db)
+        ops.cast_f32_bf16_segments(self.acc32, P.grad, [(t.storage_offset() - self.acc32.storage_offset(), P.offsets[k][0], t.numel())
+                                                        for k, t in accs.items()])
         ops.copy2d(self.dgate, G("gate"), nb, 1, 1, 8)
-
-    def _t(self, w2d):
-        return ops.transpose(w2d.contiguous())
 
     def _dw(self, dy, x, out=None):
         return ops.gemm_tn(dy, x, out=out, split=0)
@@ -1297,8 +1271,7 @@
             if k == len(fch) - 1:
                 self._query_grad()
 
-        return (schedule.pipeline_forward(head, fch, llm_fwd, lambda: (llm.HS, self.pos1, batch["proprio"], self.Np, noise), turn_around,
-                                          refresh=True)
+        return (schedule.pipeline_forward(head, fch, llm_fwd, lambda: (llm.HS, self.pos1, batch["proprio"], self.Np, noise), turn_around)
                 + schedule.pipeline_backward(head, fch, llm_bwd, lambda: self._dHS)
                 + [Segment("H", head.bwd_end, None, ("end", 0))])
 
diff --git a/vla_adapter_amd/native.py b/vla_adapter_amd/native.py
--- a/vla_adapter_amd/native.py
+++ b/vla_adapter_amd/native.py
@@ -216,9 +216,19 @@
     "an entry point belongs to one header"
 ALL_FAMILIES = FAMILIES + LATER_FAMILIES + ADDED_FAMILIES
 
+HEAD_FAMILIES = (
+    Family("head_dx", "vla_head_dx.h", {
+        "vla_gemm_bf16_nn": ([_P, C.POINTER(GemmDesc)], _I),
+        "vla_cast_f32_bf16_segments": ([_P, _P, _P, _P, _I], _I),
+    }),
+)
+HEAD_PROTOS = {name: sig for fam in HEAD_FAMILIES for name, sig in fam.protos.items()}
+assert not set(HEAD_PROTOS) & (set(PROTOS) | set(LATER_PROTOS) | set(ADDED_PROTOS)), "an entry point belongs to one header"
+REGISTRY = ALL_FAMILIES + HEAD_FAMILIES
+
 
 def family(key: str) -> Family:
-    return next(fam for fam in ALL_FAMILIES if fam.key == key)
+    return next(fam for fam in REGISTRY if fam.key == key)
 
 
 _lib = None
@@ -233,7 +243,7 @@
             f"{LIB_PATH} not found: build it with `python -c 'import __graft_entry__ as g; g.build()'` "
             f"(or `make -C {os.path.join(_HERE, 'csrc')}`).  There is no CPU/PyTorch fallback.")
     lib = C.CDLL(LIB_PATH)
-    for name, (args, res) in [sig for fam in ALL_FAMILIES for sig in fam.protos.items()]:
+    for name, (args, res) in [sig for fam in REGISTRY for sig in fam.protos.items()]:
         fn = getattr(lib, name, None)
         if fn is None:
             raise NativeLibraryMissing(f"{LIB_PATH} does not export {name}: it was built from an older source tree, rebuild (make -C csrc)")
diff --git a/vla_adapter_amd/ops.py b/vla_adapter_amd/ops.py
--- a/vla_adapter_amd/ops.py
+++ b/vla_adapter_amd/ops.py
@@ -36,13 +36,14 @@
             want_pre: bool = True, a_group=None, c_group=None, r_group=None, rope=None, c_live=None,
             split_k: Optional[int] = None, bias_post_round: bool = False, fp8=None, ext=None, query_256: bool = False,
             query_plan: bool = False):
+    nn = b.stride(-1) != 1
     if fp8 is not None:
         assert a.dtype == torch.uint8 and b.dtype == torch.uint8 and a.dim() == 2 and split_k in (None, 0, 1)
         _chk_bf16(bias, residual, out, out2)
         split_k = 0
     else:
         _chk_bf16(a, b, bias, residual, out, out2)
-    assert a.stride(-1) == 1 and b.stride(-1) == 1
+    assert a.stride(-1) == 1 and (b.stride(-2) == 1 if nn else b.stride(-1) == 1)
     batched = a.dim() == 3
     if batched:
         nb, M, K = a.shape
@@ -54,7 +55,7 @@
     assert b.shape[-1] == K, f"K mismatch {a.shape} x {b.shape}"
     d = N.GemmDesc()
     d.A, d.B = a.data_ptr(), b.data_ptr()
-    d.M, d.N, d.K, d.lda, d.ldb, d.batch = M, Nn, K, a.stride(-2), b.stride(-2), nb
+    d.M, d.N, d.K, d.lda, d.ldb, d.batch = M, Nn, K, a.stride(-2), b.stride(-1 if nn else -2), nb
     d.sA, d.sB, d.act, d.alpha, d.res_mod = sA, sB, act, alpha, res_mod
     shape = (nb, M, Nn) if batched else (M, Nn)
     if act == ACT_SWIGLU:
@@ -112,8 +113,11 @@
     if split_k and split_k > 1:
         d.split_k, d.ws = split_k, _scratch_f32(split_k * M * Nn, a.device).data_ptr()
     if query_plan or query_256:
-        plan = _nt_plan(d)
+        plan = (N.KERNEL_NT_128x128, _nt_plan(d)[1]) if nn else _nt_plan(d)
         return plan if query_plan else plan[0] == N.KERNEL_NT_256
+    if nn:
+        N.check(_lib().vla_gemm_bf16_nn(_st(), C.byref(d)), "gemm_bf16_nn")
+        return out
     N.check(_lib().vla_gemm_bf16_nt(_st(), C.byref(d)), "gemm_bf16_nt")
     if act == ACT_SWIGLU:
         return out, out2
@@ -129,6 +133,22 @@
 
 def gemm_plan(a: torch.Tensor, b: torch.Tensor, **kw) -> Tuple[int, int]:
     return gemm_nt(a, b, query_plan=True, **kw)
+
+
+def gemm_nn(a: torch.Tensor, w: torch.Tensor, **kw):
+    assert w.stride(-1) == 1 and w.shape[-1] > 1
+    return gemm_nt(a, w.transpose(-1, -2), **kw)
+
+
+def cast_f32_bf16_segments(x: torch.Tensor, y: torch.Tensor, table):
+    assert x.is_cuda and x.dtype == torch.float32 and x.is_contiguous() and y.dtype == BF16 and y.is_contiguous()
+    for s, dd, n in table:
+        assert 0 <= s and s + n <= x.numel() and 0 <= dd and dd + n <= y.numel() and n > 0, f"segment {(s, dd, n)} outside its buffers"
+    for i in range(0, len(table), 32):
+        part = [int(v) for seg in table[i:i + 32] for v in seg]
+        arr = (C.c_longlong * len(part))(*part)
+        N.check(_lib().vla_cast_f32_bf16_segments(_st(), _p(x), _p(y), arr, len(part) // 3), "cast_f32_bf16_segments")
+    return y
 
 
 class latency_hint:
diff --git a/vla_adapter_amd/trainers.py b/vla_adapter_amd/trainers.py
--- a/vla_adapter_amd/trainers.py
+++ b/vla_adapter_amd/trainers.py
@@ -340,7 +340,7 @@
         def fwd_end():
             self._pred = head.fwd_end()
         segs += schedule.pipeline_forward(head, lch, lambda c, lo, hi: llm.fwd_layers(lo, hi),
-                                          lambda: (llm.HS, eng.pos1, batch["proprio"], eng.Np, noise), fwd_end, refresh=True)
+                                          lambda: (llm.HS, eng.pos1, batch["proprio"], eng.Np, noise), fwd_end)
         self._n_forward = len(segs)
 
         def h_loss():
```
